# Ipsedo/MARLClassification

Hardware: AMD Instinct MI355X
Metric: agent-env-steps/sec (higher is better)
Workload: dtype f32; 1 GPU; RESISC45 256x256x3, 16 agents, 16 steps, f=12, README dims (configs[2]); full train iteration: rollout + A2C loss + BPTT backward + Adam; batch_per_gpu=256, global_batch=256, parallelism=dp1, rng=library (Philox4x32-10), launch=eager

## Files before the change

marlclassification_amd/csrc/common.h:

```cpp
#pragma once

#include <hip/hip_runtime.h>
#include <stdint.h>
#include <stdio.h>

#include "../../include/marl_hip.h"
#include "../../include/marl_hip_gemmops.h"
#include "split.h"

namespace marl {

constexpr int kWave = 64;

inline int p4(int x) { return (x + 3) & ~3; }
inline int64_t cdiv(int64_t a, int64_t b) { return (a + b - 1) / b; }

void set_error(const char* fmt, ...);

int tune_get(const char* key, int dflt);
int tune_set(const char* key, int value);

__device__ __forceinline__ float rcp_fast(float x) { return __builtin_amdgcn_rcpf(x); }
__device__ __forceinline__ float sigmoid_acc(float x) { return rcp_fast(1.0f + __expf(-x)); }
__device__ __forceinline__ float tanh_fast(float x) { return 1.0f - 2.0f * rcp_fast(1.0f + __expf(2.0f * x)); }
// ... 375 lines not shown
                         const float* c_prev, const float* c_new, int ldc, int64_t rows, int n,
                         hipStream_t st);
struct LstmBwdBatch;
int launch_lstm_cell_bwd_batch(LstmBwdBatch& b, int count, hipStream_t st);
int launch_lstm_cell_bwd2(const float* dh0, int lddh0, float* dc0, int lddc0, float* gates0,
                          int ldg0, const float* cp0, const float* cn0, int ldc0, int n0,
                          const float* dh1, int lddh1, float* dc1, int lddc1, float* gates1,
                          int ldg1, const float* cp1, const float* cn1, int ldc1, int n1,
                          int64_t rows, hipStream_t st);

struct SampleArgs {
    const float* a_pol;
    int ld_a, nla;
    const float* w1;
    int ldw;
    const float* b1;
    const float* noise;
    uint64_t rng_seed, rng_ctr;
    const uint64_t* rng_off_dev;
    int rng_on;
    const int64_t* forced;
    const int32_t* pos_in;
    int32_t* pos_out;
    int64_t* step_pos;
    int64_t* step_actions;
    float* step_logp;
    float* probs;
    int32_t* actions_i32;
    int R, nA, H, W, f;
    int32_t table[MARL_MAX_ACTIONS][2];
    const float* pe_W;
    const float* pe_b;
    const float* pe_gamma;
    const float* pe_beta;
    float* pe_npos;
    float* pe_z;
    float* pe_stats;
    float* pe_out;
    int pe_ldz, pe_ldo, pe_nd;
    char* pe_img;
    int pe_row0, pe_steps, pe_col0;
    float ex_inv_tau, ex_keep, ex_floor;
    int ex_greedy;
};
int launch_sample(const SampleArgs& a, hipStream_t st, bool explore = false);

int launch_draw_episode(uint64_t seed, uint64_t offset, const uint64_t* offset_dev, int64_t* pos0,
                        int R, int H, int W, int f, float* h0, float* c0, int n_b, float* hc0,
                        float* cc0, int n_a, float* noise, int64_t n_noise, hipStream_t st);

struct PermDesc {
    const float* src;
    float* dst;
    int rows, cols;
    int dst_ld;
    int rd, rs1, rs2;
    int cd, cs1, cs2;
    int frag;
    const float* src2;
};
constexpr int kMaxPerm = 56;
struct PermBatch {
    PermDesc d[kMaxPerm];
    int count;
};
int launch_permute(const PermBatch& b, hipStream_t st);

__host__ __device__ inline int panel_frag_groups(int K) { return (K + 15) >> 4; }
__host__ __device__ inline size_t panel_frag_floats(int n, int K) {
    return ((size_t)((n + 31) >> 5) * panel_frag_groups(K) + 3) * 512;
}
__host__ __device__ inline size_t panel_frag_index(int r, int k, int groups) {
    return ((((size_t)(r >> 5) * groups + (k >> 4)) * 2 + ((r >> 4) & 1)) * 64 + ((k >> 2) & 3) * 16 + (r & 15)) * 4 +
           (k & 3);
}

struct Counters {
    uint64_t rng_offset;
    uint64_t step;
    float lr_over_bc1;
    float inv_sqrt_bc2;
    float pad[2];
};
static_assert(sizeof(Counters) == MARL_COUNTERS_BYTES, "counter block layout");
int launch_counters_set(Counters* c, uint64_t rng_offset, int64_t step, float lr, float beta1,
                        float beta2, int tick, hipStream_t st);

int launch_adam(float* p, const float* g, float* m, float* v, int64_t n, float lr_over_bc1,
                float inv_sqrt_bc2, float beta1, float beta2, float eps, float grad_scale,
                hipStream_t st, const Counters* cnt = nullptr);

int launch_fill(float* p, int64_t n, float v, hipStream_t st);
int launch_add2d(const float* a, int64_t lda, const float* b, int64_t ldb, float* out, int64_t ldo,
                 int64_t rows, int cols, hipStream_t st);
int launch_copy2d(const float* src, int64_t lds, float* dst, int64_t ldd, int64_t rows, int cols,
                  hipStream_t st);
int launch_i64_to_i32(const int64_t* src, int32_t* dst, int64_t n, hipStream_t st);
int launch_policy_dlogits(const float* dlogp, const float* probs, const int32_t* actions,
                          float* out, int ld, int64_t rows, int nA, hipStream_t st);
int launch_policy_dlogits_probs(const float* dlogp, const float* dprobs, const float* probs,
                                const int32_t* actions, float* out, int ld, int64_t rows, int nA,
                                hipStream_t st);
int launch_policy_dlogits_explore(const float* dlogp, const float* dprobs, const float* probs,
                                  const int32_t* actions, float* out, int ld, int64_t rows, int nA,
                                  float inv_tau, float keep, float floor, hipStream_t st);
int launch_acc2d(float* dst, int64_t ldd, const float* src, int64_t lds, int64_t rows, int cols,
                 hipStream_t st);
int launch_rowdot(const float* a, int lda, const float* w, const float* b, float* out,
                  int64_t rows, int n, hipStream_t st);

struct PanelLayer {
    const float* wfrag;
    int wgroups;
    const float* bias;
    const float* gamma;
    const float* beta;
    int n;
    float* z;
    int ldz;
    float* stats;
    float* a;
    int lda;
    char* a3;
    int a3_row0, a3_steps, a3_col0;
};
constexpr int kPanelMaxLayers = 4;
struct PanelFwdProb {
    const float* x;
    int ldx, k0;
    int agg_na, agg_nb;
    float* xbar;
    int m, nlayers;
    PanelLayer layer[kPanelMaxLayers];
    int by_batch, g_na, g_nb, agg_at, ld_xbar;
    const float* mix;
    CommGate gate;
};
struct PanelFwdBatch {
    PanelFwdProb p[2];
    int count;
    int off_panel1, off_red, off_part, off_prm;
    int off_mix;
    int has_sample, panel_blocks;
    int epi_prob;
    int ln_narrow_max;
    SampleArgs sample;
#ifdef MARL_KERNEL_TS
    long long* ts;
#endif
};
int panel_chain_supported(int na, int n_msg, int threads);
int panel_supported(int k0, int n0, int n1);
int panel_sample_supported(int n_actions);
int launch_panel_fwd(PanelFwdBatch& b, hipStream_t st, bool explore = false);

struct LstmBwdArgs {
    const float* dh;
    float* dc;
    float* gates;
    const float* c_prev;
    const float* c_new;
    int lddh, lddc, ldg, ldc, n;
    char* g3;
    int g3_row0, g3_steps;
    int skip_f32;
};
struct LstmBwdBatch {
    LstmBwdArgs a[2];
    int64_t rows;
    int vec4;
};
inline bool lstm_bwd_vec4_ok(const LstmBwdArgs& a) {
    return (a.n & 3) == 0 && (a.lddh & 3) == 0 && (a.lddc & 3) == 0 && (a.ldg & 3) == 0 && (a.ldc & 3) == 0;
}
__device__ __forceinline__ void lstm_cell_bwd_at(const LstmBwdArgs& A, int64_t r, int u, float dhv);
__device__ __forceinline__ void lstm_cell_bwd_elem(const LstmBwdArgs& A, int64_t rows, int64_t idx) {
    const int n = A.n;
    if (idx >= rows * n) return;
    const int64_t r = idx / n;
    const int u = (int)(idx % n);
    lstm_cell_bwd_at(A, r, u, A.dh[r * A.lddh + u]);
}
__device__ __forceinline__ void lstm_cell_bwd_at(const LstmBwdArgs& A, int64_t r, int u, float dhv) {
    const int n = A.n;
    float* g = A.gates + r * A.ldg + u;
    const float gi = g[0], gf = g[n], gg = g[2 * n], go = g[3 * n];
    const float tc = tanh_fast(A.c_new[r * A.ldc + u]);
    const float dcv = dhv * go * (1.0f - tc * tc) + A.dc[r * A.lddc + u];
    g[0] = dcv * gg * gi * (1.0f - gi);
    g[n] = dcv * A.c_prev[r * A.ldc + u] * gf * (1.0f - gf);
    g[2 * n] = dcv * gi * (1.0f - gg * gg);
    g[3 * n] = dhv * tc * go * (1.0f - go);
    A.dc[r * A.lddc + u] = dcv * gf;
}

__device__ __forceinline__ void lstm_cell_bwd_at4(const LstmBwdArgs& A, int64_t r, int u, const float (&dhv)[4]) {
    const int n = A.n;
    float* g = A.gates + r * A.ldg + u;
    const float4 gi4 = *reinterpret_cast<const float4*>(g), gf4 = *reinterpret_cast<const float4*>(g + n),
                 gg4 = *reinterpret_cast<const float4*>(g + 2 * n), go4 = *reinterpret_cast<const float4*>(g + 3 * n);
    const float4 cn4 = *reinterpret_cast<const float4*>(A.c_new + r * A.ldc + u),
                 cp4 = *reinterpret_cast<const float4*>(A.c_prev + r * A.ldc + u),
                 dc4 = *reinterpret_cast<const float4*>(A.dc + r * A.lddc + u);
    const float gi[4] = {gi4.x, gi4.y, gi4.z, gi4.w}, gf[4] = {gf4.x, gf4.y, gf4.z, gf4.w};
    const float gg[4] = {gg4.x, gg4.y, gg4.z, gg4.w}, go[4] = {go4.x, go4.y, go4.z, go4.w};
    const float cn[4] = {cn4.x, cn4.y, cn4.z, cn4.w}, cp[4] = {cp4.x, cp4.y, cp4.z, cp4.w};
    const float dcin[4] = {dc4.x, dc4.y, dc4.z, dc4.w};
    float o[5][4];
#pragma unroll
    for (int q = 0; q < 4; ++q) {
        const float tc = tanh_fast(cn[q]);
        const float dcv = dhv[q] * go[q] * (1.0f - tc * tc) + dcin[q];
        o[0][q] = dcv * gg[q] * gi[q] * (1.0f - gi[q]);
        o[1][q] = dcv * cp[q] * gf[q] * (1.0f - gf[q]);
        o[2][q] = dcv * gi[q] * (1.0f - gg[q] * gg[q]);
        o[3][q] = dhv[q] * tc * go[q] * (1.0f - go[q]);
        o[4][q] = dcv * gf[q];
    }
    if (!(A.g3 && A.skip_f32)) {
#pragma unroll
        for (int k = 0; k < 4; ++k)
            *reinterpret_cast<float4*>(g + k * n) = make_float4(o[k][0], o[k][1], o[k][2], o[k][3]);
    }
    *reinterpret_cast<float4*>(A.dc + r * A.lddc + u) = make_float4(o[4][0], o[4][1], o[4][2], o[4][3]);
    if (A.g3) {
#pragma unroll
        for (int k = 0; k < 4; ++k) {
            const int col = k * n + u;
            img_store4(A.g3 + img_off(A.g3_row0 + r, col >> 4, A.g3_steps), col, o[k][0], o[k][1], o[k][2], o[k][3]);
        }
    }
}
__device__ __forceinline__ void lstm_cell_bwd_elem4(const LstmBwdArgs& A, int64_t rows, int64_t idx) {
    const int n4 = A.n >> 2;
    if (idx >= rows * n4) return;
    const int64_t r = idx / n4;
    const int u = (int)(idx - r * n4) * 4;
    const float4 d = *reinterpret_cast<const float4*>(A.dh + r * A.lddh + u);
    const float dhv[4] = {d.x, d.y, d.z, d.w};
    lstm_cell_bwd_at4(A, r, u, dhv);
}

struct PanelBwdLayer {
    const float* z;
    int ldz;
    const float* stats;
    const float* gamma;
    const float* beta;
    int n;
    float* dz;
    int lddz;
    float* part;
    const float* wtfrag;
    int wgroups;
    int k_in;
};
struct PanelBwdProb {
    const float* da;
    int ldda;
    const float* da2;
    int ldda2;
    int agg_na, agg_nb;
    int m, nlayers;
    PanelBwdLayer layer[kPanelMaxLayers];
    float* dx;
    int lddx, accumulate;
    int by_batch, g_na, g_nb, agg_at;
    int has_cellb;
    LstmBwdArgs cellb;
    int off_e, off_prm, off_colp, off_part, off_rowmap;
    const float* mix;
    int off_mix;
    int tail_lds;
    int has_cell, panel_blocks;
    LstmBwdArgs cell;
    int64_t cell_rows;
    int cell_vec4;
    int cellb_img_done, cell_img_done;
    CommGate gate;
#ifdef MARL_KERNEL_TS
    long long* ts;
#endif
};
int panel_bwd_blocks(int m);
int panel_chain_blocks(int na, int nb);
int panel_chain_by_batch(int na);
int launch_panel_bwd(PanelBwdProb& p, hipStream_t st);

#ifdef MARL_KERNEL_TS
constexpr int kTsWaves = 16, kTsSlots = 48, kTsRoles = 2;
#define MARL_TS_DECL(ptr) long long* ts_ = (ptr); int tsi_ = 0
#define MARL_TS()                                                                              \
    if (ts_ && (threadIdx.x & 63) == 0 && blockIdx.x == 37 && blockIdx.y < kTsRoles && tsi_ < kTsSlots) \
    ts_[((int)blockIdx.y * kTsWaves + (threadIdx.x >> 6)) * kTsSlots + tsi_++] = wall_clock64()
int ts_begin(long long** dev, int call);
void ts_report(const char* tag, long long* dev, int waves, int role = 0);
#else
#define MARL_TS_DECL(ptr)
#define MARL_TS()
#endif

struct FDiv {
    uint32_t d, m;
};
inline FDiv make_fdiv(int d) { return FDiv{(uint32_t)d, (uint32_t)(((1ull << 32) / (uint64_t)d) + 1)}; }
__device__ __forceinline__ int fdiv(int n, FDiv f) {
// ... 178 lines not shown
```

marlclassification_amd/csrc/episode.hip:

```cpp
#include <math.h>
#include <stdlib.h>
#include <string.h>

#include "../../include/marl_hip_rowops.h"
#include "../../include/marl_hip_cnnops.h"
#include "../../include/marl_hip_explore.h"
#include "../../include/marl_hip_classloss.h"
#include "../../include/marl_hip_softtargets.h"
#include "common.h"

namespace marl {

struct Dims {
    int na, nb, ns;
    int64_t R, NR;
    int H, W, c_img, f;
    int L;
    int ch[MARL_MAX_CNN_LAYERS + 1];
    int grp[MARL_MAX_CNN_LAYERS];
    int hw[MARL_MAX_CNN_LAYERS + 1];
    int P[MARL_MAX_CNN_LAYERS];
    int K[MARL_MAX_CNN_LAYERS];
    int ldk[MARL_MAX_CNN_LAYERS];
    int nf, nin;
// ... 399 lines not shown
    e.u3_stride_rows = 0;
    e.tn_cell[0] = e.tn_cell[1] = GemmPlan{};
    if (e.g3) {
        e.tn_cell[0] = g3_tn_cell_plan(4 * d.n_b, d.nin, d.n_b, d.NR);
        e.tn_cell[1] = g3_tn_cell_plan(4 * d.n_a, d.nin, d.n_a, d.NR);
        e.u3_stride_rows = train ? R : 0;
        e.U3 = b.take(img_bytes((int64_t)(train ? NR : R), d.nin) / sizeof(float));
        e.H3 = b.take(img_bytes((int64_t)(S1 * R), d.n_b) / sizeof(float));
        e.HC3 = b.take(img_bytes((int64_t)(S1 * R), d.n_a) / sizeof(float));
    }
    if (train && e.g3) {
        e.GB3 = b.take(img_bytes((int64_t)NR, 4 * d.n_b) / sizeof(float));
        e.GA3 = b.take(img_bytes((int64_t)NR, 4 * d.n_a) / sizeof(float));
    }
    if (train) {
        e.GPRED = b.take(NR * d.ld_nC);
        e.DLOG = b.take(NR * d.ld_nA);
        e.DVAL = b.take(NR * 4);
        e.DAQ1 = b.take(NR * d.ld_nlb);
        e.DAC1 = b.take(NR * d.ld_nla);
        e.DAP1 = b.take(NR * d.ld_nla);
        e.DH = b.take(S1 * R * d.ld_nb);
        e.DHC = b.take(S1 * R * d.ld_na);
        e.DC = b.take(R * d.ld_nb);
        e.DCC = b.take(R * d.ld_na);
        e.DDBAR = b.take(NR * d.ld_dbl);
        e.DDBAR2 = b.take(NR * d.ld_dbl);
        e.DAD1 = b.take(NR * d.ld_nm2);
        e.DMBAR = b.take(R * d.ld_nm);
        e.DZE2 = b.take(NR * d.ld_nm);
        e.DAE1 = b.take(NR * d.ld_nm2);
        e.DU = b.take(NR * d.ld_nin);
        e.DZPOS = b.take(NR * d.ld_nd);
        int maxg = 4 * (d.n_b > d.n_a ? d.n_b : d.n_a);
        e.BTMP = b.take((size_t)maxg);
        {
            int blocks = panel_bwd_blocks((int)d.R);
            if (panel_chain_blocks(d.na, d.nb) > blocks) blocks = panel_chain_blocks(d.na, d.nb);
            const size_t nblk = (size_t)blocks * d.ns * 2;
            e.PLN[0] = b.take(nblk * d.n_mo);
            e.PLN[1] = b.take(nblk * d.nm2);
            e.PLN[2] = b.take(nblk * d.n_m);
            e.PLN[3] = b.take(nblk * d.nm2);
        }
        for (int l = 0; l < d.L; ++l) {
            e.DZ[l] = b.take(NR * d.P[l] * d.ch[l + 1]);
            e.DCOLS[l] = (l > 0 && !e.dgrad[l].rb) ? b.take(NR * d.P[l] * d.ldk[l]) : 0;
            e.DA[l] = (l + 1 < d.L && !e.dgrad[l + 1].rb) ? b.take(NR * d.P[l] * d.ch[l + 1]) : 0;
        }
        size_t part = 0, tns = 0, red = 0;
        auto upd_part = [&](int64_t blocks, int n) {
            const size_t v = (size_t)blocks * 2 * n;
            part = v > part ? v : part;
            red += ((v + 63) & ~(size_t)63) + 64 * 2 * (size_t)n + 64;
        };
        auto upd_tn = [&](int ni, int nj, int64_t rows) {
            const size_t v = gemm_tn_scratch_bytes(ni, nj, rows);
            tns = v > tns ? v : tns;
            red += v / sizeof(float) + 64 * ((size_t)ni * nj + ni) + 192;
        };
        const int64_t nr = d.NR, r = d.R;
        upd_part(ln_bwd_blocks(nr, d.nlb), d.nlb);
        upd_part(ln_bwd_blocks(nr, d.nla), d.nla);
        upd_part(ln_bwd_blocks(nr, d.n_d), d.n_d);
        upd_part(ln_bwd_blocks(r, d.nm2), d.nm2);
        upd_part(ln_bwd_blocks(r, d.n_mo), d.n_mo);
        upd_part(ln_bwd_blocks(r, d.n_m), d.n_m);
        for (int l = 0; l < d.L; ++l) upd_part(gn_bwd_blocks(nr, d.ch[l + 1]), d.ch[l + 1]);
        for (int l = 1; l < d.L; ++l)
            if (e.dgrad[l].rb) upd_part(e.dgrad[l].chunks, d.ch[l]);
        upd_tn(d.nC, d.nlb, nr);
        upd_tn(d.nlb, d.n_b, nr);
        upd_tn(1, d.nla, nr);
        upd_tn(d.nla, d.n_a, nr);
        upd_tn(d.nA, d.nla, nr);
        upd_tn(d.n_mo, d.nm2, nr);
        upd_tn(d.nm2, d.n_m, nr);
        upd_tn(d.n_m, d.nm2, nr);
        upd_tn(d.nm2, d.n_b, nr);
        upd_tn(4 * d.n_b, d.nin, nr);
        upd_tn(4 * d.n_b, d.n_b, nr);
        upd_tn(4 * d.n_a, d.nin, nr);
        upd_tn(4 * d.n_a, d.n_a, nr);
        if (e.g3) {
            const int tn3[4][2] = {{4 * d.n_b, d.nin}, {4 * d.n_b, d.n_b}, {4 * d.n_a, d.nin}, {4 * d.n_a, d.n_a}};
            for (const auto& q : tn3) {
                const size_t v = g3_tn_plan(q[0], q[1], nr, false).scratch_bytes;
                tns = v > tns ? v : tns;
            }
            for (const GemmPlan& q : e.tn_cell) tns = q.scratch_bytes > tns ? q.scratch_bytes : tns;
        }
        upd_tn(d.n_d, 2, nr);
        for (int l = 0; l < d.L; ++l) {
            if (e.wgrad[l].form) {
                const size_t v = (size_t)e.wgrad[l].blocks_bound *
                                 ((size_t)d.ch[l + 1] * d.K[l] + d.ch[l + 1]) * sizeof(float);
                tns = v > tns ? v : tns;
                red += v / sizeof(float) + 64 * ((size_t)d.ch[l + 1] * (d.K[l] + 1)) + 192;
            } else {
                upd_tn(d.ch[l + 1], d.K[l], nr * d.P[l]);
            }
        }
        e.part_floats = part;
        e.tns_bytes = tns;
        e.PART = b.take(part);
        e.TNS = b.take(tns / sizeof(float) + 16);
        {
            const int pn[4] = {d.n_mo, d.nm2, d.n_m, d.nm2};
            for (int n : pn) red += 64 * 2 * (size_t)n + 64;
        }
        e.red_floats = red + 4096;
        e.RED = b.take(e.red_floats);
    }
    e.loss_floats = loss_scratch_floats(d.ns, d.na, d.nb);
    e.LOSS = b.take(e.loss_floats);
    e.total = b.off;
}

struct Explore {
    bool on;
    float inv_tau, keep, eps;
    int greedy;
};
struct ClassLoss {
    bool on;
    const float* w;
    int nc;
    float eps;
    const float* sw;
    int ns;
    bool wrew;
};
struct SoftTargets {
    const float* q;
    int nb, nc;
};
struct Installed {
    const float* comm = nullptr;
    int comm_na = 0;
    CommGate range = {nullptr, -1, 0, 1};
    Explore explore = {false, 1.f, 1.f, 0.f, 0};
    ClassLoss class_loss = {false, nullptr, 0, 0.f, nullptr, 0, false};
    SoftTargets soft = {nullptr, 0, 0};
    hipEvent_t heads_event = nullptr;
};
static Installed g_installed;

enum SampleSite { SAMPLE_OWN = 0, SAMPLE_EPILOGUE, SAMPLE_RIDE };
struct Plan {
    bool panels;
    bool panels_bwd;
    bool chain;
    bool panel_sample;
    bool g3_lstm;
    bool g3_tn, g3_tn_pipe;
    bool g3_tn_cell;
    bool u3_by_producers;
    int skip_f32;
    int lstm_plan;
    SampleSite sample;
    int comm_form;
    int explore_form;
    int comm, comm_range, explore, class_loss;
    int soft_targets;
};

struct Ctx {
    Dims d;
    WLayout w;
    ELayout e;
    float* W;
    float* E;
    hipStream_t st;
    int train;
    RedQueue* rq = nullptr;
    TnQueue* tq = nullptr;
    bool defer_slabs = false;
    size_t defer_small = 0;
    bool defer_this(size_t slab_bytes) const { return defer_slabs || (defer_small && slab_bytes <= defer_small); }
    Installed opt;
    Plan plan;
    int u3_row(int t) const { return (int)(e.u3_stride_rows * (size_t)t); }

    const char* wp3k(int i) const { return reinterpret_cast<const char*>(W + w.wp3k[i]); }
    const char* wt3k(int i) const { return reinterpret_cast<const char*>(W + w.wt3k[i]); }
    char* img(size_t off) const { return reinterpret_cast<char*>(E + off); }
    const float* wp(int i) const { return W + w.wp[i]; }
    const float* wt(int i) const { return W + w.wt[i]; }
    GemmB wpB(int i) const {
        const ParamMeta m = param_meta(d, i);
        return GemmB{wp(i), w.ldp[i], m.k, m.kind == PK_MATRIX ? W + w.wp3[i] : nullptr, (m.k + 31) / 32};
    }
    GemmB wtB(int i) const {
        const ParamMeta m = param_meta(d, i);
        return GemmB{wt(i), w.ldt[i], m.n, m.kind == PK_MATRIX ? W + w.wt3[i] : nullptr, (m.n + 31) / 32};
    }
    const float* wpf(int i) const { return w.wpf[i] ? W + w.wpf[i] : nullptr; }
    const float* wtf(int i) const { return w.wtf[i] ? W + w.wtf[i] : nullptr; }
    float* gp(int i) const { return W + w.gp[i]; }
    float* at(size_t off) const { return E + off; }
    float* at(const SBuf& s, int t) const { return E + s.at(train ? t : 0); }
    float* Hs(int t) const { return E + e.H + (size_t)t * d.R * d.ld_nb; }
    float* Cs(int t) const { return E + e.C + (size_t)t * d.R * d.ld_nb; }
    float* HCs(int t) const { return E + e.HC + (size_t)t * d.R * d.ld_na; }
    float* CCs(int t) const { return E + e.CC + (size_t)t * d.R * d.ld_na; }
    float* MSGs(int t) const { return E + e.MSG + (size_t)t * d.R * d.ld_nm; }
    int32_t* POSs(int t) const { return reinterpret_cast<int32_t*>(E + e.POS) + (size_t)t * d.R * 2; }
    float* PROBSs(int t) const { return E + e.PROBS + (size_t)t * d.R * d.nA; }
    int32_t* ACTs(int t) const { return reinterpret_cast<int32_t*>(E + e.ACT) + (size_t)t * d.R; }
    float* DHs(int t) const { return E + e.DH + (size_t)t * d.R * d.ld_nb; }
    float* DHCs(int t) const { return E + e.DHC + (size_t)t * d.R * d.ld_na; }
};

static Plan make_plan(const Dims& d, const WLayout& w, const ELayout& e, const Installed& opt) {
    auto env_on = [](const char* v) { return !(v && v[0] == '0'); };
    static const bool env_panels = env_on(getenv("MARL_PANELS")), env_sample = env_on(getenv("MARL_PANEL_SAMPLE"));
    Plan p{};
    p.panels = env_panels && panel_model_ok(d);
    p.panels_bwd = p.panels && d.n_mo <= 384 && d.nm2 <= 384 && d.n_m <= 384;
    p.chain = p.panels_bwd && panel_chain_supported(d.na, d.n_m, 256) && tune_get("panel_chain", 1) != 0 &&
              (!opt.comm || d.n_b <= 384);
    p.panel_sample = p.chain && env_sample && panel_sample_supported(d.nA);
    p.sample = p.chain ? (p.panel_sample ? SAMPLE_EPILOGUE : SAMPLE_OWN)
                       : (p.panels && !opt.explore.on ? SAMPLE_RIDE : SAMPLE_OWN);
    p.comm_form = opt.comm ? (p.chain ? 5 : p.panels ? 3 : 4) : p.chain ? 0 : p.panels ? 1 : 2;
    p.explore_form = !opt.explore.on ? 0 : p.panel_sample ? 1 : 2;
    p.comm = opt.comm != nullptr;
    p.comm_range = opt.range.radius >= 0 ? opt.range.radius : -1;
    p.explore = opt.explore.on;
    p.class_loss = opt.class_loss.on;
    p.soft_targets = opt.soft.q != nullptr;

    const int k_lstm = tune_get("g3_lstm", 1), k_tn = tune_get("g3_tn", 1);
    p.g3_lstm = e.g3 && k_lstm != 0;
    if (p.g3_lstm) {
        G3Batch b{};
        b.count = 2;
        b.p[0].m = b.p[1].m = (int)d.R;
        b.p[0].n = d.n_b;
        b.p[1].n = d.n_a;
        p.lstm_plan = g3_lstm_plan(b).variant;
    }
    p.g3_tn = p.g3_lstm && k_tn != 0 &&
              (k_tn == 2 || (d.nin <= 640 && d.n_b <= 512 && d.n_a <= 512 &&
                             (d.NR >= 32768 || (e.tn_cell[0].ok && e.tn_cell[1].ok))));
    p.g3_tn_cell = p.g3_tn && e.tn_cell[0].ok && e.tn_cell[1].ok;
    p.g3_tn_pipe = p.g3_tn && e.tn_cell[0].pipelined;
    p.skip_f32 = p.panels_bwd && p.g3_tn;
    p.u3_by_producers = p.g3_lstm && e.fwd.writes_image && p.panels &&
                        ((d.nf | d.n_mo | d.n_d) & 3) == 0 &&
                        d.nin % 16 == 0;
    return p;
}

static int make_ctx(const marl_config* cfg, const void* wws, size_t wbytes, void* ews, size_t ebytes,
                    int train, void* stream, Ctx& c) {
    MARL_TRY(make_dims(cfg, c.d));
    c.opt = g_installed;
    if (c.opt.comm && c.opt.comm_na != c.d.na) {
        set_error("communication matrix is %d x %d but the configuration has %d agents", c.opt.comm_na,
                  c.opt.comm_na, c.d.na);
        return MARL_EINVAL;
    }
    if (c.opt.range.radius >= 0 && !c.opt.comm) {
        set_error("a communication range is installed without its base matrix (marl_comm_matrix)");
        return MARL_EINVAL;
    }
    make_wlayout(c.d, c.w);
    make_elayout(c.d, c.w, train, c.e);
    if (wbytes < c.w.total * sizeof(float) || ebytes < c.e.total * sizeof(float)) {
        set_error("workspace too small for the current configuration / tuning knobs: weights %zu of %zu "
                  "bytes, episode %zu of %zu bytes (ask marl_workspace_sizes again)", wbytes,
                  c.w.total * sizeof(float), ebytes, c.e.total * sizeof(float));
        return MARL_ESIZE;
    }
    c.W = const_cast<float*>(static_cast<const float*>(wws));
    c.E = static_cast<float*>(ews);
    c.st = static_cast<hipStream_t>(stream);
    c.train = train;
    if (!c.W || !c.E) {
        set_error("null workspace");
        return MARL_EINVAL;
    }
    if ((reinterpret_cast<uintptr_t>(c.W) & 255) || (reinterpret_cast<uintptr_t>(c.E) & 255)) {
        set_error("workspaces must be 256-byte aligned");
        return MARL_EINVAL;
    }
    c.plan = make_plan(c.d, c.w, c.e, c.opt);
    return MARL_OK;
}

static int gemm1(const Ctx& c, const GemmProb& p) {
    GemmBatch b{};
    b.p[0] = p;
    b.count = 1;
    return launch_gemm_nt(b, c.st);
}
static int gemm2(const Ctx& c, const GemmProb& p0, const GemmProb& p1) {
    GemmBatch b{};
    b.p[0] = p0;
    b.p[1] = p1;
    b.count = 2;
    return launch_gemm_nt(b, c.st);
}

struct StepIn {
    const float* obs = nullptr;
    const float* npos = nullptr;
    const void* img = nullptr;
    int img_u8 = 0;
};

struct CnnFwdIo {
    const void* img = nullptr;
    const float* obs = nullptr;
    const int32_t* pos = nullptr;
    int img_u8 = 0;
    int64_t rows = 0;
    float* cols[MARL_MAX_CNN_LAYERS] = {};
    float* z[MARL_MAX_CNN_LAYERS] = {};
    float* gst[MARL_MAX_CNN_LAYERS] = {};
    float* u = nullptr;
    int ldu = 0;
    char* u3 = nullptr;
    int u3_row0 = 0, u3_steps = 0;
};
static CnnFwdArgs cnn_fwd_args(const Dims& d, const WLayout& w, const float* W, const CnnFwdIo& io) {
    CnnFwdArgs a{};
    a.img = io.img;
    a.obs = io.obs;
    a.pos = io.pos;
    a.img_u8 = io.img_u8;
    a.rows = io.rows;
    a.nb = d.nb;
    a.c_img = d.c_img;
    a.H = d.H;
    a.W = d.W;
    a.f = d.f;
    a.L = d.L;
    for (int l = 0; l < d.L; ++l)
        a.layer[l] = CnnFwdLayer{W + w.wp[4 * l], W + w.wp[4 * l + 1], W + w.wp[4 * l + 2], W + w.wp[4 * l + 3],
                                 io.cols[l], io.z[l], io.gst[l],
                                 d.ch[l], d.ch[l + 1], d.grp[l], d.hw[l], d.hw[l + 1], d.P[l],
                                 d.K[l], d.ldk[l], w.wf[4 * l] ? W + w.wf[4 * l] : nullptr};
    a.u = io.u;
    a.ldu = io.ldu;
    a.u3 = io.u3;
    a.u3_row0 = io.u3_row0;
    a.u3_steps = io.u3_steps;
    return a;
}


static int step_cnn(const Ctx& c, int t, const StepIn& in) {
    const Dims& d = c.d;
    hipStream_t st = c.st;
    if (c.e.fwd.which) {
        CnnFwdIo io;
        io.img = in.img;
        io.obs = in.obs;
        io.pos = c.POSs(t);
        io.img_u8 = in.img_u8;
        io.rows = d.R;
        for (int l = 0; l < d.L; ++l) {
            io.cols[l] = c.e.keeps_cols[l] ? c.at(c.e.COLS[l], t) : nullptr;
            io.z[l] = c.train ? c.at(c.e.Z[l], t) : nullptr;
            io.gst[l] = c.train ? c.at(c.e.GST[l], t) : nullptr;
        }
        io.u = c.at(c.e.U, t);
        io.ldu = d.ld_nin;
        if (c.plan.u3_by_producers) {
            io.u3 = c.img(c.e.U3);
            io.u3_row0 = c.u3_row(t);
            io.u3_steps = img_steps(d.nin);
        }
// ... 1865 lines not shown
                       size_t step_ws_bytes, const float* obs, const float* g_probs, const float* g_logp,
                       const float* g_values, const float* g_preds, const float* g_msg, const float* g_h,
                       const float* g_c, const float* g_hc, const float* g_cc, float* const* grads_host,
                       float* d_msg, float* d_h, float* d_c, float* d_hc, float* d_cc, void* stream) {
    if (!cfg) {
        set_error("step_backward: null configuration");
        return MARL_EINVAL;
    }
    if (g_installed.range.radius >= 0) {
        set_error("step_backward: a communication range is installed - a single step has no integer positions of "
                  "the emission step; run the fused episode");
        return MARL_EINVAL;
    }
    marl_config one = *cfg;
    one.nb_steps = 1;
    Ctx c;
    MARL_TRY(make_ctx(&one, weights_ws, weights_ws_bytes, step_ws, step_ws_bytes, 1, stream, c));
    if (!grads_host || !obs) {
        set_error("step_backward: null gradient table or observation");
        return MARL_EINVAL;
    }
    StepBwd sb;
    sb.obs = obs;
    sb.g_probs = g_probs;
    sb.g_msg = g_msg;
    sb.g_h = g_h;
    sb.g_c = g_c;
    sb.g_hc = g_hc;
    sb.g_cc = g_cc;
    sb.d_msg = d_msg;
    sb.d_h = d_h;
    sb.d_c = d_c;
    sb.d_hc = d_hc;
    sb.d_cc = d_cc;
    return episode_backward(c, nullptr, 0, g_preds, g_logp, g_values, grads_host, &sb);
}

int marl_debug_buffer(const marl_config* cfg, int train, const char* name, int t,
                      int64_t* offset_floats, int* ld) {
    Dims d;
    MARL_TRY(make_dims(cfg, d));
    WLayout w;
    make_wlayout(d, w);
    ELayout e;
    make_elayout(d, w, train, e);
    if (!name || !offset_floats || !ld || t < 0 || t > d.ns) return MARL_EINVAL;
    const size_t R = (size_t)d.R;
    const int ts = train ? t : 0;
    auto set = [&](size_t off, int l) {
        *offset_floats = (int64_t)off;
        *ld = l;
        return MARL_OK;
    };
    if (!strncmp(name, "WP", 2) || !strncmp(name, "WT", 2)) {
        const int idx = atoi(name + 2);
        if (name[2] == 'F') {
            const int fi = atoi(name + 3);
            const size_t off = fi >= 0 && fi < MARL_NPARAMS ? (name[1] == 'P' ? w.wpf[fi] : w.wtf[fi]) : 0;
            if (!off) {
                set_error("parameter %d has no fragment-order copy", fi);
                return MARL_EINVAL;
            }
            return set(off, name[1] == 'P' ? w.gpf[fi] : w.gtf[fi]);
        }
        if (idx < 0 || idx >= MARL_NPARAMS || param_meta(d, idx).kind == PK_NONE) {
            set_error("no parameter %d", idx);
            return MARL_EINVAL;
        }
        return name[1] == 'P' ? set(w.wp[idx], w.ldp[idx]) : set(w.wt[idx], w.ldt[idx]);
    }
    if (!strcmp(name, "U")) return set(e.U.at(ts), d.ld_nin);
    if (!strcmp(name, "H")) return set(e.H + (size_t)t * R * d.ld_nb, d.ld_nb);
    if (!strcmp(name, "C")) return set(e.C + (size_t)t * R * d.ld_nb, d.ld_nb);
    if (!strcmp(name, "HC")) return set(e.HC + (size_t)t * R * d.ld_na, d.ld_na);
    if (!strcmp(name, "CC")) return set(e.CC + (size_t)t * R * d.ld_na, d.ld_na);
    if (!strcmp(name, "MSG")) return set(e.MSG + (size_t)t * R * d.ld_nm, d.ld_nm);
    if (!strcmp(name, "PROBS")) return set(e.PROBS + (size_t)t * R * d.nA, d.nA);
    if (!strcmp(name, "COLS0")) {
        if (e.fwd.which && !e.keeps_cols[0]) {
            set_error("COLS0 is not materialised for this shape (fused CNN kernels)");
            return MARL_EINVAL;
        }
        return set(e.COLS[0].at(e.COLS[0].stride ? ts : 0), d.ldk[0]);
    }
    if (!strcmp(name, "Z0")) return set(e.Z[0].at(ts), d.ch[1]);
    if (!strcmp(name, "GB")) return set(e.GB.at(ts), d.ld_gb);
    if (train) {
        if (!strcmp(name, "DU")) return set(e.DU + (size_t)t * R * d.ld_nin, d.ld_nin);
        if (!strcmp(name, "DH")) return set(e.DH + (size_t)t * R * d.ld_nb, d.ld_nb);
        if (!strcmp(name, "DHC")) return set(e.DHC + (size_t)t * R * d.ld_na, d.ld_na);
    }
    set_error("unknown debug buffer %s", name);
    return MARL_EINVAL;
}

int marl_plan_query(const marl_config* cfg, int train, const char* key, int* value) {
    Dims d;
    MARL_TRY(make_dims(cfg, d));
    if (!key || !value) return MARL_EINVAL;
    WLayout w;
    make_wlayout(d, w);
    ELayout e;
    make_elayout(d, w, train, e);
    const Plan plan = make_plan(d, w, e, g_installed);
    if (!strcmp(key, "g3")) *value = e.g3;
    else if (!strcmp(key, "g3_model")) *value = g3_model_ok(d);
    else if (!strcmp(key, "g3_lstm")) *value = plan.g3_lstm;
    else if (!strcmp(key, "g3_tn")) *value = plan.g3_tn;
    else if (!strcmp(key, "lstm_plan")) *value = plan.lstm_plan;
    else if (!strcmp(key, "small_r")) *value = plan.lstm_plan == 3 || plan.lstm_plan == 4;
    else if (!strcmp(key, "g3_tn_cell"))
        *value = plan.g3_tn_cell;
    else if (!strcmp(key, "g3_tn_pipe")) *value = plan.g3_tn_pipe;
    else if (!strcmp(key, "wgrad3")) {
        *value = 0;
        for (int l = 0; l < d.L; ++l)
            if (e.wgrad[l].form == 3) *value = 1;
    }
    else if (!strncmp(key, "cnn_fwd", 7)) {
        const CnnFwdPlan& p = e.fwd;
        if (!strcmp(key, "cnn_fwd")) *value = p.which;
        else if (!strcmp(key, "cnn_fwd_rb")) *value = p.rb;
        else if (!strcmp(key, "cnn_fwd_blocks")) *value = p.blocks;
        else {
            set_error("unknown plan key %s", key);
            return MARL_EINVAL;
        }
    }
    else if (!strncmp(key, "cnn_dgrad_rb", 12) || !strncmp(key, "cnn_wgrad_", 10)) {
        const bool dg = key[4] == 'd';
        const char* rest = key + (dg ? 12 : 10);
        int field = 0;
        if (!dg) {
            if (!strncmp(rest, "rb", 2)) field = 1, rest += 2;
            else if (!strncmp(rest, "chunks", 6)) field = 2, rest += 6;
            else if (!strncmp(rest, "blocks", 6)) field = 3, rest += 6;
        }
        const int l = (rest[0] >= '0' && rest[0] <= '9' && !rest[1]) ? rest[0] - '0' : -1;
        if ((!dg && !field) || l < (dg ? 1 : 0) || l >= d.L) {
            set_error("unknown plan key %s (layers %d..%d)", key, dg ? 1 : 0, d.L - 1);
            return MARL_EINVAL;
        }
        if (dg)
            *value = e.dgrad[l].rb;
        else {
            const CnnWgradPlan& p = e.wgrad[l];
            *value = field == 1 ? p.rb : field == 2 ? p.chunks : p.blocks;
        }
    }
    else if (!strcmp(key, "comm")) *value = plan.comm;
    else if (!strcmp(key, "comm_range")) *value = plan.comm_range;
    else if (!strcmp(key, "panel_chain")) *value = plan.chain;
    else if (!strcmp(key, "panel_sample")) *value = plan.panel_sample;
    else if (!strcmp(key, "explore")) *value = plan.explore;
    else if (!strcmp(key, "class_loss")) *value = plan.class_loss;
    else if (!strcmp(key, "soft_targets")) *value = plan.soft_targets;
    else if (!strcmp(key, "explore_form")) *value = plan.explore_form;
    else if (!strcmp(key, "comm_form")) *value = plan.comm_form;
    else {
        set_error("unknown plan key %s", key);
        return MARL_EINVAL;
    }
    return MARL_OK;
}

}
namespace marl {
__global__ void normalize_positions_kernel(const int64_t* __restrict__ pos, float* __restrict__ out,
                                           int rows, int H, int W) {
    const int r = blockIdx.x * blockDim.x + threadIdx.x;
    if (r >= rows) return;
    out[r * 2] = (float)pos[r * 2] / (float)H;
    out[r * 2 + 1] = (float)pos[r * 2 + 1] / (float)W;
}
}
extern "C" {

int marl_normalize_positions(const int64_t* pos, float* out, int rows, int h, int w, void* stream) {
    if (!pos || !out || rows < 1 || h < 1 || w < 1) {
        set_error("normalize_positions: bad argument");
        return MARL_EINVAL;
    }
    hipLaunchKernelGGL(normalize_positions_kernel, dim3((unsigned)cdiv(rows, 256)), dim3(256), 0,
                       static_cast<hipStream_t>(stream), pos, out, rows, h, w);
    MARL_LAUNCH_CHECK();
    return MARL_OK;
}

int marl_profile_begin(int kernel_class, int max_launches) {
    if (kernel_class < 0 || kernel_class >= kProfClasses || max_launches < 1) return MARL_EINVAL;
    return profile_begin(kernel_class, max_launches);
}
int marl_profile_end(double* total_ms, int* launches) { return profile_end(total_ms, launches); }

int marl_gemm_nt(const float* a, int lda, const float* b, int ldb, const float* bias, float* c,
                 int ldc, int m, int n, int k, int accumulate, void* stream) {
    GemmBatch bt{};
    bt.p[0] = gemm_prob(a, lda, gemm_b(b, ldb, k), c, ldc, m, n, bias, accumulate);
    bt.count = 1;
    return launch_gemm_nt(bt, static_cast<hipStream_t>(stream));
}

size_t marl_gemm_weight_image_bytes(int n, int k) { return split_image_floats(n, k) * sizeof(float); }

int marl_gemm_nt_weights(const float* a, int lda, const float* b, int ldb, const float* bias, float* c,
                         int ldc, int m, int n, int k, int accumulate, void* image_scratch, void* stream) {
    if (!b || !image_scratch || n < 1 || k < 1 || ldb < k) {
        set_error("gemm_nt_weights: bad argument");
        return MARL_EINVAL;
    }
    hipStream_t st = static_cast<hipStream_t>(stream);
    SplitBatch sb{};
    sb.d[0] = SplitDesc{b, image_scratch, n, k, ldb, (k + 31) / 32};
    sb.count = 1;
    MARL_TRY(launch_split_weights(sb, st));
    GemmBatch bt{};
    bt.p[0] = gemm_prob(a, lda, GemmB{b, ldb, k, image_scratch, (k + 31) / 32}, c, ldc, m, n, bias, accumulate);
    bt.count = 1;
    return launch_gemm_nt(bt, st);
}

size_t marl_gemm_tn_scratch(int ni, int nj, int64_t rows) { return gemm_tn_scratch_bytes(ni, nj, rows); }

int marl_gemm_tn(const float* a, int lda, const float* b, int ldb, float* c, int ldc, int ni, int nj,
                 int64_t rows, float* scratch, size_t scratch_bytes, void* stream) {
    return launch_gemm_tn(a, lda, b, ldb, c, ldc, ni, nj, rows, scratch, scratch_bytes,
                          static_cast<hipStream_t>(stream));
}

static CnnWgradArgs wgrad_api_args(int64_t rows, int nb, int c_img, int h, int w, int cin, int cout,
                                   int hin, int groups, int first) {
    CnnWgradArgs g{};
    g.rows = rows;
    g.first = first;
    g.nb = nb;
    g.c_img = c_img;
    g.H = h;
    g.W = w;
    g.cin = cin;
    g.cout = cout;
    g.hin = hin;
    g.hout = (hin - 1) / 2 + 1;
    g.P = g.hout * g.hout;
    g.G = groups > 0 ? groups : 1;
    g.K = 9 * cin;
    return g;
}

size_t marl_cnn_wgrad_scratch(int64_t rows, int cin, int cout, int hin, int groups, int first) {
    CnnWgradArgs g = wgrad_api_args(rows, 1, cin, hin + 1, hin + 1, cin, cout, hin, groups, first);
    return (size_t)cnn_wgrad_plan(g).blocks_bound * ((size_t)cout * 9 * cin + cout) * sizeof(float);
}

int marl_cnn_wgrad(const float* dz, const void* img, int img_u8, const int32_t* pos,
                   const float* zin, const float* gst, const float* gamma, const float* beta,
                   int64_t rows, int nb, int c_img, int h, int w, int cin, int cout, int hin,
                   int groups, float* dw, float* db, float* scratch, size_t scratch_bytes,
                   void* stream) {
    const int first = zin == nullptr;
    if (!dz || !dw || !db || !scratch || rows < 1 || cin < 1 || cout < 1 || hin < 1 ||
        (first ? (!img || !pos || nb < 1) : (!gst || !gamma || !beta))) {
        set_error("cnn_wgrad: bad argument");
        return MARL_EINVAL;
    }
    CnnWgradArgs g = wgrad_api_args(rows, nb, c_img, h, w, cin, cout, hin, groups, first);
    const CnnWgradPlan plan = cnn_wgrad_plan(g);
    if (!plan.form) {
        set_error("cnn_wgrad: shape outside the kernel's range (cin %d cout %d hin %d)", cin, cout, hin);
        return MARL_ELIMIT;
    }
    if (scratch_bytes < (size_t)plan.blocks_bound * ((size_t)cout * 9 * cin + cout) * sizeof(float)) {
        set_error("cnn_wgrad: scratch too small");
        return MARL_ESIZE;
    }
    g.dz = dz;
    g.img = img;
    g.img_u8 = img_u8;
    g.pos = pos;
    g.zin = zin;
    g.gst = gst;
    g.gamma = gamma;
    g.beta = beta;
    g.part_w = scratch;
    hipStream_t st = static_cast<hipStream_t>(stream);
    MARL_TRY(launch_cnn_wgrad(g, st));
    return launch_slab_reduce(g.part_w, (int64_t)cout * g.K, g.blocks, dw, g.K, cout, g.K, g.part_b, db, st);
}

int marl_tune(const char* key, int value) {
    if (!key) return MARL_EINVAL;
    return tune_set(key, value);
}

int marl_tune_get(const char* key, int dflt) { return key ? tune_get(key, dflt) : dflt; }

int marl_ln_silu_fwd(const float* z, int ldz, const float* gamma, const float* beta, float* out,
                     int ldo, float* stats, int m, int n, void* stream) {
    return launch_ln_silu_fwd(z, ldz, gamma, beta, out, ldo, stats, m, n,
                              static_cast<hipStream_t>(stream));
}

int marl_ln_silu_bwd(const float* da, int ldda, const float* g, int ldg, int kin, const float* w1t, int ldw,
                     const float* z, int ldz, const float* stats, const float* gamma, const float* beta,
                     float* dz, int lddz, float* dgamma, float* dbeta, float* scratch, size_t scratch_bytes,
                     int m, int n, void* stream) {
    if (!z || !stats || !gamma || !beta || !dz || !dgamma || !dbeta || !scratch || m < 0 || n < 1 ||
// ... 209 lines not shown
```

marlclassification_amd/csrc/panel.hip:

```cpp
#include <stdlib.h>

#include "common.h"
#include "sample.h"

namespace marl {

typedef float f32x4 __attribute__((ext_vector_type(4)));

__device__ __forceinline__ void lds_barrier() {
    asm volatile("s_waitcnt lgkmcnt(0)\n\ts_barrier" ::: "memory");
}
__device__ __forceinline__ float silu_p(float y) { return silu_fast(y); }
__device__ __forceinline__ float silu_grad_p(float y) { return silu_grad_fast(y); }

constexpr int kPanelRows = 16;
constexpr int kPanelMaxWaves = 12;
constexpr int kPanelMaxCols = 6;

__host__ __device__ inline int panel_stride(int k) { return ((k + 15) & ~15) + 4; }

__device__ __forceinline__ void panel_gemm(f32x4 (&acc)[2], const float* in, int stride,
                                           const float* __restrict__ wfrag, int groups, int j,
                                           int kbeg, int kend, int lane) {
    const int quad = lane >> 4, l16 = lane & 15;
    const float* arow = in + l16 * stride + 4 * quad;
    const int g0 = __builtin_amdgcn_readfirstlane(j * groups + (kbeg >> 4));
    const float* wb = wfrag + (size_t)g0 * 512;
    const unsigned lo = 4u * (unsigned)lane;
#pragma unroll
    for (int r = 0; r < 4; ++r) acc[0][r] = acc[1][r] = 0.f;
    for (int k0 = kbeg; k0 < kend; k0 += 64, wb += 4 * 512) {
        float4 b0[4], b1[4];
#pragma unroll
        for (int i = 0; i < 4; ++i) {
            b0[i] = *reinterpret_cast<const float4*>(wb + 512 * i + lo);
            b1[i] = *reinterpret_cast<const float4*>(wb + 512 * i + 256 + lo);
        }
#pragma unroll
        for (int i = 0; i < 4; ++i) {
            if (k0 + 16 * i < kend) {
                const float4 a = *reinterpret_cast<const float4*>(arow + k0 + 16 * i);
                acc[0] = __builtin_amdgcn_mfma_f32_16x16x4f32(a.x, b0[i].x, acc[0], 0, 0, 0);
                acc[1] = __builtin_amdgcn_mfma_f32_16x16x4f32(a.x, b1[i].x, acc[1], 0, 0, 0);
                acc[0] = __builtin_amdgcn_mfma_f32_16x16x4f32(a.y, b0[i].y, acc[0], 0, 0, 0);
                acc[1] = __builtin_amdgcn_mfma_f32_16x16x4f32(a.y, b1[i].y, acc[1], 0, 0, 0);
                acc[0] = __builtin_amdgcn_mfma_f32_16x16x4f32(a.z, b0[i].z, acc[0], 0, 0, 0);
                acc[1] = __builtin_amdgcn_mfma_f32_16x16x4f32(a.z, b1[i].z, acc[1], 0, 0, 0);
                acc[0] = __builtin_amdgcn_mfma_f32_16x16x4f32(a.w, b0[i].w, acc[0], 0, 0, 0);
                acc[1] = __builtin_amdgcn_mfma_f32_16x16x4f32(a.w, b1[i].w, acc[1], 0, 0, 0);
            }
        }
    }
}

__device__ __forceinline__ void panel_ksum(f32x4 (&acc)[2], float* part, int nt, int ks, int j, int s,
                                           int lane, bool active) {
    if (ks > 1) {
        if (active && s > 0) {
            float* p = part + ((size_t)((s - 1) * nt + j) * 64 + lane) * 8;
            *reinterpret_cast<float4*>(p) = make_float4(acc[0][0], acc[0][1], acc[0][2], acc[0][3]);
            *reinterpret_cast<float4*>(p + 4) = make_float4(acc[1][0], acc[1][1], acc[1][2], acc[1][3]);
        }
        lds_barrier();
        if (active && s == 0) {
            for (int q = 1; q < ks; ++q) {
                const float* p = part + ((size_t)((q - 1) * nt + j) * 64 + lane) * 8;
                const float4 u = *reinterpret_cast<const float4*>(p);
                const float4 v = *reinterpret_cast<const float4*>(p + 4);
                acc[0][0] += u.x;
                acc[0][1] += u.y;
                acc[0][2] += u.z;
                acc[0][3] += u.w;
                acc[1][0] += v.x;
                acc[1][1] += v.y;
                acc[1][2] += v.z;
                acc[1][3] += v.w;
            }
        }
    }
}

__host__ __device__ inline int panel_ksplit(int K, int nt, int nwaves) {
    const int K16 = (K + 15) & ~15;
    int ks = nwaves / nt;
    const int want = (K16 + 63) / 64;
    ks = ks < want ? ks : want;
    return ks < 1 ? 1 : ks;
}

template <int NC>
__device__ __forceinline__ void panel_ln_rows(const PanelLayer& Lr, float* outp, int ys, int n, const float* lgamma,
                                              const float* lbeta, const int* rowmap, int wave, int nwaves, int lane)
{
    constexpr int RPW = 4;
    float g[NC], bt[NC];
#pragma unroll
    for (int u = 0; u < NC; ++u) {
        const int c = lane + 64 * u;
        g[u] = c < n ? lgamma[c] : 0.f;
        bt[u] = c < n ? lbeta[c] : 0.f;
    }
    const float inv_n = 1.0f / (float)n;
#pragma unroll
    for (int i = 0; i < RPW; ++i) {
        const int lr = wave + i * nwaves;
        if (lr < kPanelRows) {
            float* zr = outp + lr * ys;
            const int row = rowmap[lr];
            float v[NC];
            float sm = 0.f;
#pragma unroll
            for (int u = 0; u < NC; ++u) {
                const int c = lane + 64 * u;
                v[u] = c < n ? zr[c] : 0.f;
                sm += v[u];
                if (Lr.z && row >= 0 && c < n) Lr.z[(size_t)row * Lr.ldz + c] = v[u];
            }
            const float mean = wave_sum(sm) * inv_n;
            float q = 0.f;
#pragma unroll
            for (int u = 0; u < NC; ++u) {
                const int c = lane + 64 * u;
                const float d = c < n ? v[u] - mean : 0.f;
                v[u] = d;
                q += d * d;
            }
            const float rstd = 1.0f / sqrtf(wave_sum(q) * inv_n + 1e-5f);
            float* arow = Lr.a + (size_t)(row < 0 ? 0 : row) * Lr.lda;
#pragma unroll
            for (int u = 0; u < NC; ++u) {
                const int c = lane + 64 * u;
                if (c < n) {
                    const float av = silu_p(v[u] * rstd * g[u] + bt[u]);
                    zr[c] = av;
                    if (row >= 0) arow[c] = av;
                }
            }
            if (Lr.stats && lane == 0 && row >= 0) {
                Lr.stats[(size_t)row * 2] = mean;
                Lr.stats[(size_t)row * 2 + 1] = rstd;
            }
            if (Lr.a3 && row >= 0) {
                for (int c4 = 4 * lane; c4 < n; c4 += 256) {
                    const float4 t = *reinterpret_cast<const float4*>(zr + c4);
                    const int col = Lr.a3_col0 + c4;
                    img_store4(Lr.a3 + img_off((int64_t)Lr.a3_row0 + row, col >> 4, Lr.a3_steps), col, t.x, t.y, t.z, t.w);
                }
            }
        }
    }
}

template <int MAXA, bool UNI, bool EXPLORE = false>
__device__ __forceinline__ void panel_sample_rows(const SampleArgs& A0, const float* outp, int ys, const int* rowmap,
                                                  int wave, int nwaves, int lane) {
    for (int lr = __builtin_amdgcn_readfirstlane(wave); lr < kPanelRows; lr += nwaves) {
        const int row = __builtin_amdgcn_readfirstlane(rowmap[lr]);
        if (row < 0) continue;
        int ln = (int)__builtin_amdgcn_mbcnt_hi(~0u, __builtin_amdgcn_mbcnt_lo(~0u, 0u));
        asm volatile("" : "+v"(ln));
        int zero = 0;
        asm volatile("" : "+s"(zero));
        const SampleArgs& A = (&A0)[zero];
        float p[MAXA];
        SamplePre<MAXA> S;
        sample_prefetch_row<MAXA>(A, row, ln, S);
        sample_row_logits_at<MAXA, kPanelMaxCols>(A, outp + lr * ys, p, ln);
        if (UNI) {
            auto uni = [](float v) { return __int_as_float(__builtin_amdgcn_readfirstlane(__float_as_int(v))); };
#pragma unroll
            for (int j = 0; j < MAXA; ++j) {
                S.b1[j] = uni(S.b1[j]);
                S.nz[j] = uni(S.nz[j]);
            }
            S.ctr = ((uint64_t)(uint32_t)__builtin_amdgcn_readfirstlane((int)(S.ctr >> 32)) << 32) |
                    (uint32_t)__builtin_amdgcn_readfirstlane((int)S.ctr);
            S.pi0 = __builtin_amdgcn_readfirstlane(S.pi0);
            S.pi1 = __builtin_amdgcn_readfirstlane(S.pi1);
            S.forced = __builtin_amdgcn_readfirstlane(S.forced);
        }
        sample_prefetch_pe<MAXA>(A, ln, S);
        sample_finish<MAXA, EXPLORE>(A, row, p, ln, S);
    }
}

template <int SAMPLE, bool MIX = false, bool EPI = false, bool GATE = false, bool EXPLORE = false>
__global__ __launch_bounds__(768, 6) void panel_fwd_kernel(const PanelFwdBatch B) {
    extern __shared__ __attribute__((aligned(16))) float lds[];
    if (!EPI && SAMPLE > 0 && (int)blockIdx.x >= B.panel_blocks) {
        const int r = ((int)blockIdx.x - B.panel_blocks) * (int)(blockDim.x >> 6) + (int)(threadIdx.x >> 6);
        if (r >= B.sample.R) return;
        constexpr int MAXA = SAMPLE > 0 ? SAMPLE : 4;
        float p[MAXA];
        SamplePre<MAXA> S;
        sample_prefetch<MAXA, false>(B.sample, r, threadIdx.x & 63, S);
        sample_row_logits<MAXA>(B.sample, r, p, threadIdx.x & 63);
        sample_finish<MAXA>(B.sample, r, p, threadIdx.x & 63, S);
        return;
    }
    const PanelFwdProb& P = B.p[blockIdx.y];
    const int m0 = blockIdx.x * kPanelRows;
    const int bpb = P.by_batch;
    if (bpb ? (int)blockIdx.x * bpb >= P.g_nb : m0 >= P.m) return;
    const int tid = threadIdx.x, lane = tid & 63, wave = tid >> 6, nwaves = blockDim.x >> 6;
    int* rowmap = reinterpret_cast<int*>(lds + B.off_red);
    if (tid < kPanelRows) {
        int r = m0 + tid < P.m ? m0 + tid : -1;
        if (bpb) {
            const int a = tid / bpb, b = (int)blockIdx.x * bpb + (tid - a * bpb);
            r = (a < P.g_na && b < P.g_nb) ? a * P.g_nb + b : -1;
        }
        rowmap[tid] = r;
    }
    lds_barrier();
    const int quad = lane >> 4, l16 = lane & 15;
#ifdef MARL_KERNEL_TS
    MARL_TS_DECL(B.ts);
#endif
    MARL_TS();
    float* X = lds;
    float* Y = lds + B.off_panel1;
    float* part = lds + B.off_part;
    float* prm = lds + B.off_prm;
    float pv[kPanelMaxLayers][3];
#pragma unroll
    for (int l = 0; l < kPanelMaxLayers; ++l) {
        pv[l][0] = pv[l][1] = pv[l][2] = 0.f;
        if (l < P.nlayers && tid < P.layer[l].n) {
            pv[l][0] = P.layer[l].bias[tid];
            pv[l][1] = P.layer[l].gamma[tid];
            pv[l][2] = P.layer[l].beta[tid];
        }
    }
    float cmv = 0.f;
    if (MIX && !GATE && P.mix && tid < P.g_na * P.g_na) cmv = P.mix[tid];
    if (MIX && GATE && tid < bpb * P.g_na * P.g_na) {
        const int na = P.g_na, i = tid / (na * na), e = tid - i * na * na, a = e / na;
        const int b = (int)blockIdx.x * bpb + i;
        if (b < P.g_nb) cmv = comm_gate_weight<kPanelRows>(P.mix, P.gate, na, P.g_nb, b, a, e - a * na);
    }

    {
        const int k0 = P.k0, xs = panel_stride(k0), K16 = (k0 + 15) & ~15;
        const int c4 = K16 >> 2;
        const int K4 = (k0 + 3) & ~3;
        if (!GATE && P.agg_na > 0) {
            const int na = P.agg_na, nb = P.agg_nb;
            const float den = (float)(na - 1);
            for (int e = tid; e < kPanelRows * c4; e += blockDim.x) {
                const int lr = e / c4, k = (e % c4) * 4;
                const int r = rowmap[lr];
                float4 v = make_float4(0.f, 0.f, 0.f, 0.f);
                if (r >= 0 && k < K4 && na > 1) {
                    const int b = r % nb;
                    const float* base = P.x + (size_t)b * P.ldx + k;
                    const size_t astr = (size_t)nb * P.ldx;
                    float4 s = make_float4(0.f, 0.f, 0.f, 0.f);
                    for (int a0 = 0; a0 < na; a0 += 8) {
                        float4 qv[8];
#pragma unroll
                        for (int u = 0; u < 8; ++u) {
                            const int a = a0 + u < na ? a0 + u : na - 1;
                            qv[u] = *reinterpret_cast<const float4*>(base + (size_t)a * astr);
                        }
#pragma unroll
                        for (int u = 0; u < 8; ++u) {
                            if (a0 + u < na) {
                                s.x += qv[u].x;
                                s.y += qv[u].y;
                                s.z += qv[u].z;
                                s.w += qv[u].w;
                            }
                        }
                    }
                    const float4 me = *reinterpret_cast<const float4*>(P.x + (size_t)r * P.ldx + k);
                    v = make_float4((s.x - me.x) / den, (s.y - me.y) / den, (s.z - me.z) / den,
                                    (s.w - me.w) / den);
                    if (P.xbar) *reinterpret_cast<float4*>(P.xbar + (size_t)r * P.ldx + k) = v;
                }
                *reinterpret_cast<float4*>(X + lr * xs + k) = v;
            }
        } else {
            float4 xv[2];
#pragma unroll
            for (int it = 0; it < 2; ++it) {
                const int e = tid + it * (int)blockDim.x;
                xv[it] = make_float4(0.f, 0.f, 0.f, 0.f);
                if (e < kPanelRows * c4) {
                    const int lr = e / c4, k = (e % c4) * 4;
                    const int r = rowmap[lr];
                    if (r >= 0 && k < K4) xv[it] = *reinterpret_cast<const float4*>(P.x + (size_t)r * P.ldx + k);
                }
            }
#pragma unroll
            for (int it = 0; it < 2; ++it) {
                const int e = tid + it * (int)blockDim.x;
                if (e < kPanelRows * c4) {
                    const int lr = e / c4, k = (e % c4) * 4;
                    *reinterpret_cast<float4*>(X + lr * xs + k) = xv[it];
                }
            }
            for (int e = tid + 2 * (int)blockDim.x; e < kPanelRows * c4; e += blockDim.x) {
                const int lr = e / c4, k = (e % c4) * 4;
                const int r = rowmap[lr];
                float4 v = make_float4(0.f, 0.f, 0.f, 0.f);
                if (r >= 0 && k < K4) v = *reinterpret_cast<const float4*>(P.x + (size_t)r * P.ldx + k);
                *reinterpret_cast<float4*>(X + lr * xs + k) = v;
            }
        }
    }
    {
        int off = 0;
#pragma unroll
        for (int l = 0; l < kPanelMaxLayers; ++l) {
            if (l < P.nlayers) {
                const int n = P.layer[l].n;
                if (tid < n) {
                    prm[off + tid] = pv[l][0];
                    prm[off + n + tid] = pv[l][1];
                    prm[off + 2 * n + tid] = pv[l][2];
                }
                off += 3 * n;
            }
        }
    }
    if (MIX && !GATE && P.mix && tid < P.g_na * P.g_na) lds[B.off_mix + tid] = cmv;
    if (MIX && GATE && tid < bpb * P.g_na * P.g_na) lds[B.off_mix + tid] = cmv;
    MARL_TS();
    lds_barrier();
    MARL_TS();

    int prm_off = 0, K = P.k0;
    for (int l = 0; l < P.nlayers; ++l) {
        const PanelLayer Lr = P.layer[l];
        const float* lbias = prm + prm_off;
        const float* lgamma = lbias + Lr.n;
        const float* lbeta = lgamma + Lr.n;
        prm_off += 3 * Lr.n;
        float* in = (l & 1) ? Y : X;
        float* outp = (l & 1) ? X : Y;
        const int K16 = (K + 15) & ~15;
        const int stride = panel_stride(K);
        if (l > 0 && l == P.agg_at) {
            const int c4 = K16 >> 2, K4 = (K + 3) & ~3, na = P.g_na;
            const float den = (float)(na - 1);
            float4 v[2];
#pragma unroll
            for (int it = 0; it < 2; ++it) {
                const int e = tid + it * (int)blockDim.x;
                v[it] = make_float4(0.f, 0.f, 0.f, 0.f);
                if (e < kPanelRows * c4) {
                    const int lr = e / c4, k = (e - lr * c4) * 4;
                    const int a = lr / bpb, i = lr - a * bpb;
                    if (MIX) {
                        if (a < na) {
                            const float* crow = lds + B.off_mix + (GATE ? i * na + a : a) * na;
                            float4 sm = make_float4(0.f, 0.f, 0.f, 0.f);
                            for (int a2 = 0; a2 < na; ++a2) {
                                const float cf = crow[a2];
                                if (cf != 0.f) {
                                    const float4 q = *reinterpret_cast<const float4*>(in + (a2 * bpb + i) * stride + k);
                                    sm.x = fmaf(cf, q.x, sm.x);
                                    sm.y = fmaf(cf, q.y, sm.y);
                                    sm.z = fmaf(cf, q.z, sm.z);
                                    sm.w = fmaf(cf, q.w, sm.w);
                                }
                            }
                            v[it] = sm;
                        }
                    } else if (a < na && na > 1) {
                        float4 sm = make_float4(0.f, 0.f, 0.f, 0.f);
                        for (int a2 = 0; a2 < na; ++a2) {
                            const float4 q = *reinterpret_cast<const float4*>(in + (a2 * bpb + i) * stride + k);
                            sm.x += q.x;
                            sm.y += q.y;
                            sm.z += q.z;
                            sm.w += q.w;
                        }
                        const float4 me = *reinterpret_cast<const float4*>(in + lr * stride + k);
                        v[it] = make_float4((sm.x - me.x) / den, (sm.y - me.y) / den, (sm.z - me.z) / den,
                                            (sm.w - me.w) / den);
                    }
                }
            }
            lds_barrier();
#pragma unroll
            for (int it = 0; it < 2; ++it) {
                const int e = tid + it * (int)blockDim.x;
                if (e < kPanelRows * c4) {
                    const int lr = e / c4, k = (e - lr * c4) * 4;
                    *reinterpret_cast<float4*>(in + lr * stride + k) = v[it];
                    const int r = rowmap[lr];
                    if (r >= 0 && k < K4 && P.xbar)
                        *reinterpret_cast<float4*>(P.xbar + (size_t)r * P.ld_xbar + k) = v[it];
                }
            }
            lds_barrier();
        }
        const int n = Lr.n, nt = (n + 31) >> 5;
        const int ks = panel_ksplit(K, nt, nwaves);
        const int j = wave % nt, s = wave / nt;
        const bool active = s < ks;
        const int kper = (((K16 + ks - 1) / ks) + 15) & ~15;
        const int kbeg = s * kper;
        const int kend = kbeg + kper < K16 ? kbeg + kper : K16;
        f32x4 acc[2];
        if (active) panel_gemm(acc, in, stride, Lr.wfrag, Lr.wgroups, j, kbeg, kend, lane);
        MARL_TS();
        panel_ksum(acc, part, nt, ks, j, s, lane, active);
        MARL_TS();

        const int ys = panel_stride(n), n16 = (n + 15) & ~15;
        if (active && s == 0) {
#pragma unroll
            for (int t = 0; t < 2; ++t) {
                const int col = j * 32 + 16 * t + l16;
                const bool cv = col < n;
                const float bv = cv ? lbias[col] : 0.f;
#pragma unroll
                for (int r = 0; r < 4; ++r) {
                    const int lr = 4 * quad + r;
                    const float zv = cv ? acc[t][r] + bv : 0.f;
                    if (col < n16) outp[lr * ys + col] = zv;
                }
            }
        }
        MARL_TS();
        lds_barrier();
        MARL_TS();
        if (n <= B.ln_narrow_max)
            panel_ln_rows<2>(Lr, outp, ys, n, lgamma, lbeta, rowmap, wave, nwaves, lane);
        else
            panel_ln_rows<kPanelMaxCols>(Lr, outp, ys, n, lgamma, lbeta, rowmap, wave, nwaves, lane);
        MARL_TS();
        lds_barrier();
        MARL_TS();
        K = n;
    }
    if (EPI && (int)(&P - B.p) + 1 == B.epi_prob) {
        constexpr int MAXA = SAMPLE > 0 ? SAMPLE : 4;
        panel_sample_rows<MAXA, MIX || EXPLORE, EXPLORE>(B.sample, (P.nlayers & 1) ? Y : X, panel_stride(K), rowmap, wave, nwaves, lane);
        MARL_TS();
    }
}

constexpr size_t kPanelMaxLds = 144 * 1024;

static int panel_waves_for(int k, int n) {
    const int nt = (n + 31) / 32;
    const int want = (((k + 15) & ~15) + 63) / 64;
    int w = nt * want;
    if (w < nt) w = nt;
    return w > kPanelMaxWaves ? (nt > kPanelMaxWaves ? -1 : (kPanelMaxWaves / nt) * nt) : w;
}

int panel_chain_supported(int na, int n_msg, int threads) {
    const int K16 = (n_msg + 15) & ~15;
    return na >= 1 && na <= kPanelRows && kPanelRows * (K16 / 4) <= 2 * threads;
}

int panel_sample_supported(int n_actions) { return n_actions >= 1 && n_actions <= 4; }

int panel_supported(int k0, int n0, int n1) {
    if (n0 > 32 * kPanelMaxWaves || n1 > 32 * kPanelMaxWaves) return 0;
    if (n0 > 64 * kPanelMaxCols || n1 > 64 * kPanelMaxCols) return 0;
    const int kx = k0 > n1 ? k0 : n1;
    const size_t lds = (size_t)(kPanelRows * panel_stride(kx) + kPanelRows * panel_stride(n0) +
                                (kPanelMaxWaves + 1) * 32 + (kPanelMaxWaves - 1) * 512 +
                                3 * (n0 + n1) + 16) * 4;
    return lds <= kPanelMaxLds;
}

static int panel_kper_host(int K16, int ks) { return (((K16 + ks - 1) / ks) + 15) & ~15; }

struct PanelFwdPlan {
    int waves;
    size_t lds;
    unsigned pblocks;
    bool mixed, gated;
};
static int panel_fwd_plan(PanelFwdBatch& b, PanelFwdPlan& pl) {
    int waves = 1, x0 = 0, x1 = 0;
    for (int i = 0; i < b.count; ++i) {
        const PanelFwdProb& p = b.p[i];
        for (int l = 0; l < p.nlayers; ++l) {
            const int kin = l == 0 ? p.k0 : p.layer[l - 1].n;
            if (!p.layer[l].wfrag) {
                set_error("panel kernel: layer %d has no fragment-order weight copy", l);
                return MARL_EINVAL;
            }
            if (p.layer[l].wgroups != panel_frag_groups(kin)) {
                set_error("panel kernel: layer %d's weight copy has %d K groups, its input width %d needs %d", l,
                          p.layer[l].wgroups, kin, panel_frag_groups(kin));
                return MARL_ELIMIT;
            }
            const int w = panel_waves_for(kin, p.layer[l].n);
            if (w < 0) {
                set_error("panel kernel: layer width %d too large", p.layer[l].n);
                return MARL_ELIMIT;
            }
            waves = w > waves ? w : waves;
        }
        int s0 = kPanelRows * panel_stride(p.k0), s1 = 0;
        for (int l = 0; l < p.nlayers; ++l) {
            const int v = kPanelRows * panel_stride(p.layer[l].n);
            if (l & 1)
                s0 = v > s0 ? v : s0;
            else
                s1 = v > s1 ? v : s1;
        }
        if (p.agg_at > 0 && (p.by_batch < 1 || p.g_na * p.by_batch > kPanelRows || p.agg_at >= p.nlayers ||
                             !panel_chain_supported(p.g_na, p.layer[p.agg_at - 1].n, 256))) {
            set_error("panel kernel: in-panel message mean outside its range");
            return MARL_ELIMIT;
        }
        if (p.mix && (p.agg_at <= 0 || i != 0 || (b.has_sample && b.count == 1))) {
            set_error("panel kernel: a mixing matrix needs the in-panel aggregation of problem 0");
            return MARL_ELIMIT;
        }
        if ((p.gate.pos && (!p.mix || p.by_batch * p.g_na * p.g_na > kPanelRows * kPanelRows)) ||
            (b.p[0].gate.pos && p.agg_na > 0)) {
            set_error("panel kernel: a position gate needs a base matrix, no staged mean and by_batch * agents^2 <= %d",
                      kPanelRows * kPanelRows);
            return MARL_ELIMIT;
        }
        x0 = s0 > x0 ? s0 : x0;
        x1 = s1 > x1 ? s1 : x1;
    }
    const bool mixed = b.count > 0 && b.p[0].mix != nullptr;
    const bool gated = mixed && b.p[0].gate.pos != nullptr;
    if (waves < 4) waves = 4;
    b.off_panel1 = x0;
    b.off_red = x0 + x1;
    b.off_part = b.off_red + (kPanelMaxWaves + 1) * 32;
    b.off_prm = b.off_part + (waves - 1) * 512;
    int prm = 0;
    for (int i = 0; i < b.count; ++i) {
        int q = 0;
        for (int l = 0; l < b.p[i].nlayers; ++l) q += 3 * b.p[i].layer[l].n;
        prm = q > prm ? q : prm;
    }
    b.off_mix = b.off_prm + prm + 16;
    const size_t lds = (size_t)(b.off_mix + (mixed ? kPanelRows * kPanelRows : 0)) * sizeof(float);
    if (lds > kPanelMaxLds) {
        set_error("panel kernel: shape outside its range");
        return MARL_ELIMIT;
    }
    b.ln_narrow_max = 128;
    unsigned pblocks = 0;
    for (int i = 0; i < b.count; ++i) {
        const PanelFwdProb& p = b.p[i];
        const unsigned nblk = p.by_batch > 0 ? (unsigned)cdiv(p.g_nb, p.by_batch) : (unsigned)cdiv(p.m, kPanelRows);
        pblocks = nblk > pblocks ? nblk : pblocks;
    }
    pl.waves = waves;
    pl.lds = lds;
    pl.pblocks = pblocks;
    pl.mixed = mixed;
    pl.gated = gated;
    return MARL_OK;
}

int launch_panel_fwd(PanelFwdBatch& b, hipStream_t st, bool explore) {
    PanelFwdPlan pl;
    MARL_TRY(panel_fwd_plan(b, pl));
    const int waves = pl.waves;
    const size_t lds = pl.lds;
    const unsigned pblocks = pl.pblocks;
    const bool mixed = pl.mixed, gated = pl.gated;
    static bool raised = false;
    if (!raised) {
        const void* kerns[11] = {reinterpret_cast<const void*>(panel_fwd_kernel<0>),
                                reinterpret_cast<const void*>(panel_fwd_kernel<4>),
                                reinterpret_cast<const void*>(panel_fwd_kernel<MARL_MAX_ACTIONS>),
                                reinterpret_cast<const void*>(panel_fwd_kernel<0, true>),
                                reinterpret_cast<const void*>(panel_fwd_kernel<4, false, true>),
                                reinterpret_cast<const void*>(panel_fwd_kernel<4, true, true>),
                                reinterpret_cast<const void*>(panel_fwd_kernel<0, true, false, true>),
                                reinterpret_cast<const void*>(panel_fwd_kernel<4, true, true, true>),
                                reinterpret_cast<const void*>(panel_fwd_kernel<4, false, true, false, true>),
                                reinterpret_cast<const void*>(panel_fwd_kernel<4, true, true, false, true>),
                                reinterpret_cast<const void*>(panel_fwd_kernel<4, true, true, true, true>)};
        for (const void* kf : kerns)
            MARL_HIP_CHECK(hipFuncSetAttribute(kf, hipFuncAttributeMaxDynamicSharedMemorySize, (int)kPanelMaxLds));
        raised = true;
    }
#ifdef MARL_KERNEL_TS
    static long long* d_ts = nullptr;
    static int calls = 0;
    const int rec = ts_begin(&d_ts, calls++);
    b.ts = rec ? d_ts : nullptr;
#endif
    if (b.epi_prob) {
        const PanelFwdProb* p = b.epi_prob >= 1 && b.epi_prob <= b.count ? &b.p[b.epi_prob - 1] : nullptr;
        if (!p || !panel_sample_supported(b.sample.nA) || p->nlayers < 1 || p->m != b.sample.R ||
            p->layer[p->nlayers - 1].a != b.sample.a_pol || p->layer[p->nlayers - 1].n != b.sample.nla) {
            set_error("panel kernel: the sampling epilogue needs the problem whose last layer writes its activations");
            return MARL_EINVAL;
        }
    }
    if (explore && !b.epi_prob) {
        set_error("panel kernel: exploration controls are served by the sampling epilogue only");
        return MARL_EINVAL;
    }
    for (int i = 0; i < b.count; ++i) {
        const PanelFwdProb& p = b.p[i];
        if (p.agg_na == 1 && p.xbar) {
            PermBatch z{};
            z.count = 1;
            z.d[0].dst = p.xbar, z.d[0].rows = p.m, z.d[0].cols = (p.k0 + 3) & ~3, z.d[0].dst_ld = p.ldx;
            z.d[0].rd = z.d[0].cd = 1;
            MARL_TRY(launch_permute(z, st));
        }
    }
    prof_before(4, st);
    if (b.epi_prob && explore) {
        b.has_sample = 0;
        if (gated)
            hipLaunchKernelGGL((panel_fwd_kernel<4, true, true, true, true>), dim3(pblocks, (unsigned)b.count),
                               dim3(64 * waves), lds, st, b);
        else if (mixed)
            hipLaunchKernelGGL((panel_fwd_kernel<4, true, true, false, true>), dim3(pblocks, (unsigned)b.count),
                               dim3(64 * waves), lds, st, b);
        else
            hipLaunchKernelGGL((panel_fwd_kernel<4, false, true, false, true>), dim3(pblocks, (unsigned)b.count),
                               dim3(64 * waves), lds, st, b);
    } else if (b.epi_prob) {
        b.has_sample = 0;
        if (gated)
            hipLaunchKernelGGL((panel_fwd_kernel<4, true, true, true>), dim3(pblocks, (unsigned)b.count),
                               dim3(64 * waves), lds, st, b);
        else if (mixed)
            hipLaunchKernelGGL((panel_fwd_kernel<4, true, true>), dim3(pblocks, (unsigned)b.count), dim3(64 * waves),
                               lds, st, b);
        else
            hipLaunchKernelGGL((panel_fwd_kernel<4, false, true>), dim3(pblocks, (unsigned)b.count), dim3(64 * waves),
                               lds, st, b);
    } else if (b.has_sample && b.count == 1) {
        b.panel_blocks = (int)pblocks;
        const unsigned sblocks = (unsigned)cdiv(b.sample.R, waves);
        if (b.sample.nA <= 4)
            hipLaunchKernelGGL(panel_fwd_kernel<4>, dim3(pblocks + sblocks, 1), dim3(64 * waves), lds, st, b);
        else
            hipLaunchKernelGGL(panel_fwd_kernel<MARL_MAX_ACTIONS>, dim3(pblocks + sblocks, 1), dim3(64 * waves), lds, st, b);
    } else {
        b.has_sample = 0;
        if (gated)
            hipLaunchKernelGGL((panel_fwd_kernel<0, true, false, true>), dim3(pblocks, (unsigned)b.count),
                               dim3(64 * waves), lds, st, b);
        else if (mixed)
            hipLaunchKernelGGL((panel_fwd_kernel<0, true>), dim3(pblocks, (unsigned)b.count), dim3(64 * waves),
                               lds, st, b);
        else
            hipLaunchKernelGGL(panel_fwd_kernel<0>, dim3(pblocks, (unsigned)b.count), dim3(64 * waves), lds, st, b);
    }
    prof_after(4, st);
    MARL_LAUNCH_CHECK();
#ifdef MARL_KERNEL_TS
    if (rec) {
        fprintf(stderr, "[ts] panel_fwd count %d sample %d epilogue %d waves %d lds %zu\n", b.count, b.has_sample,
                b.epi_prob, waves, lds);
        ts_report("panel_fwd", d_ts, waves);
        if (b.count == 2) ts_report("panel_fwd role 1", d_ts, waves, 1);
    }
#endif
    return MARL_OK;
}

constexpr int kBwdMaxCols = kPanelMaxCols;

template <bool CELL, int MAXC, bool MIX = false, bool GATE = false>
__global__ __launch_bounds__(768, 4) void panel_bwd_kernel(const PanelBwdProb P) {
    extern __shared__ __attribute__((aligned(16))) float lds[];
    if (CELL && (int)blockIdx.x >= P.panel_blocks) {
        const int64_t idx = (int64_t)((int)blockIdx.x - P.panel_blocks) * blockDim.x + threadIdx.x;
        if (P.cell_vec4)
            lstm_cell_bwd_elem4(P.cell, P.cell_rows, idx);
        else
            lstm_cell_bwd_elem(P.cell, P.cell_rows, idx);
        return;
    }
    const int m0 = blockIdx.x * kPanelRows;
    const int bpb = P.by_batch;
    if (bpb ? (int)blockIdx.x * bpb >= P.g_nb : m0 >= P.m) return;
    const int tid = threadIdx.x, lane = tid & 63, wave = tid >> 6, nwaves = blockDim.x >> 6;
    const int quad = lane >> 4, l16 = lane & 15;
    float* D = lds;
    float* E = lds + P.off_e;
    float* prm = lds + P.off_prm;
    float* colp = lds + P.off_colp;
    float* part = lds + P.off_part;
    int* rowmap = reinterpret_cast<int*>(lds + P.off_rowmap);
    if (tid < kPanelRows) {
        int r = m0 + tid < P.m ? m0 + tid : -1;
        if (bpb) {
            const int a = tid / bpb, b = (int)blockIdx.x * bpb + (tid - a * bpb);
            r = (a < P.g_na && b < P.g_nb) ? a * P.g_nb + b : -1;
        }
        rowmap[tid] = r;
    }
    lds_barrier();
#ifdef MARL_KERNEL_TS
    MARL_TS_DECL(P.ts);
#endif
    MARL_TS();

    float zpre[2][MAXC], mpre[2], rpre[2];
    auto zfetch = [&](const PanelBwdLayer& L) {
#pragma unroll
        for (int i = 0; i < 2; ++i) {
            const int lr = wave + i * nwaves;
            const int row = lr < kPanelRows ? rowmap[lr] : -1;
            const size_t rr = row < 0 ? 0 : (size_t)row;
            mpre[i] = L.stats[rr * 2];
            rpre[i] = L.stats[rr * 2 + 1];
#pragma unroll
            for (int u = 0; u < MAXC; ++u) {
                const int c = lane + 64 * u;
                zpre[i][u] = c < L.n ? L.z[rr * L.ldz + c] : 0.f;
            }
        }
    };
    zfetch(P.layer[0]);
    {
        float pv[kPanelMaxLayers][2];
#pragma unroll
        for (int l = 0; l < kPanelMaxLayers; ++l) {
            pv[l][0] = pv[l][1] = 0.f;
            if (l < P.nlayers && tid < P.layer[l].n) {
                pv[l][0] = P.layer[l].gamma[tid];
                pv[l][1] = P.layer[l].beta[tid];
            }
        }
        float cmv = 0.f;
        if (MIX && !GATE && tid < P.g_na * P.g_na) {
            const int a = tid / P.g_na, a2 = tid - a * P.g_na;
            cmv = P.mix[a2 * P.g_na + a];
        }
        if (MIX && GATE && tid < bpb * P.g_na * P.g_na) {
            const int na = P.g_na, i = tid / (na * na), e = tid - i * na * na, a = e / na;
            const int b = (int)blockIdx.x * bpb + i;
            if (b < P.g_nb) cmv = comm_gate_weight<kPanelRows>(P.mix, P.gate, na, P.g_nb, b, e - a * na, a);
        }
        int off = 0;
#pragma unroll
        for (int l = 0; l < kPanelMaxLayers; ++l) {
            if (l < P.nlayers) {
                const int n = P.layer[l].n;
                if (tid < n) {
                    prm[off + tid] = pv[l][0];
                    prm[off + n + tid] = pv[l][1];
                }
                off += 2 * n;
            }
        }
        if (MIX && !GATE && tid < P.g_na * P.g_na) lds[P.off_mix + tid] = cmv;
        if (MIX && GATE && tid < bpb * P.g_na * P.g_na) lds[P.off_mix + tid] = cmv;
        const int n = P.layer[0].n, ds = panel_stride(n), n16 = (n + 15) & ~15, c4 = n16 >> 2;
        const int n4 = (n + 3) & ~3;
        for (int e = tid; e < kPanelRows * c4; e += blockDim.x) {
            const int lr = e / c4, k = (e % c4) * 4;
            const int r = rowmap[lr];
            float4 v = make_float4(0.f, 0.f, 0.f, 0.f);
            if (r >= 0 && k < n4 && P.agg_na > 1) {
                const int na = P.agg_na, nb = P.agg_nb;
                const float den = (float)(na - 1);
                const float* base = P.da + (size_t)(r % nb) * P.ldda + k;
                const size_t astr = (size_t)nb * P.ldda;
                float4 s = make_float4(0.f, 0.f, 0.f, 0.f);
                for (int a0 = 0; a0 < na; a0 += 8) {
                    float4 qv[8];
#pragma unroll
                    for (int u = 0; u < 8; ++u) {
                        const int a = a0 + u < na ? a0 + u : na - 1;
                        qv[u] = *reinterpret_cast<const float4*>(base + (size_t)a * astr);
                    }
#pragma unroll
                    for (int u = 0; u < 8; ++u) {
                        if (a0 + u < na) {
                            s.x += qv[u].x;
                            s.y += qv[u].y;
                            s.z += qv[u].z;
                            s.w += qv[u].w;
                        }
                    }
                }
                const float4 me = *reinterpret_cast<const float4*>(P.da + (size_t)r * P.ldda + k);
                v = make_float4((s.x - me.x) / den, (s.y - me.y) / den, (s.z - me.z) / den,
                                (s.w - me.w) / den);
            } else if (r >= 0 && k < n4 && P.agg_na == 0) {
                v = *reinterpret_cast<const float4*>(P.da + (size_t)r * P.ldda + k);
                if (P.da2) {
                    const float4 w = *reinterpret_cast<const float4*>(P.da2 + (size_t)r * P.ldda2 + k);
                    v = make_float4(v.x + w.x, v.y + w.y, v.z + w.z, v.w + w.w);
                }
            }
            *reinterpret_cast<float4*>(D + lr * ds + k) = v;
        }
    }
    MARL_TS();
    lds_barrier();
    MARL_TS();

    int prm_off = 0;
    for (int l = 0; l < P.nlayers; ++l) {
        const PanelBwdLayer Lr = P.layer[l];
        const int n = Lr.n, ds = panel_stride(n), n16 = (n + 15) & ~15;
        const float* lgamma = prm + prm_off;
        const float* lbeta = lgamma + n;
        prm_off += 2 * n;
        if (l > 0 && l == P.agg_at) {
            const int c4 = n16 >> 2, na = P.g_na;
            const float den = (float)(na - 1);
            float4 v[2];
#pragma unroll
            for (int it = 0; it < 2; ++it) {
                const int e = tid + it * (int)blockDim.x;
                v[it] = make_float4(0.f, 0.f, 0.f, 0.f);
                if (e < kPanelRows * c4) {
                    const int lr = e / c4, k = (e - lr * c4) * 4;
                    const int a = lr / bpb, i = lr - a * bpb;
                    if (MIX) {
                        if (a < na) {
                            const float* crow = lds + P.off_mix + (GATE ? i * na + a : a) * na;
                            float4 sm = make_float4(0.f, 0.f, 0.f, 0.f);
                            for (int a2 = 0; a2 < na; ++a2) {
                                const float cf = crow[a2];
                                if (cf != 0.f) {
                                    const float4 q = *reinterpret_cast<const float4*>(D + (a2 * bpb + i) * ds + k);
                                    sm.x = fmaf(cf, q.x, sm.x);
                                    sm.y = fmaf(cf, q.y, sm.y);
                                    sm.z = fmaf(cf, q.z, sm.z);
                                    sm.w = fmaf(cf, q.w, sm.w);
                                }
                            }
                            v[it] = sm;
                        }
                    } else if (a < na && na > 1) {
                        float4 sm = make_float4(0.f, 0.f, 0.f, 0.f);
                        for (int a2 = 0; a2 < na; ++a2) {
                            const float4 q = *reinterpret_cast<const float4*>(D + (a2 * bpb + i) * ds + k);
                            sm.x += q.x;
                            sm.y += q.y;
                            sm.z += q.z;
                            sm.w += q.w;
                        }
                        const float4 me = *reinterpret_cast<const float4*>(D + lr * ds + k);
                        v[it] = make_float4((sm.x - me.x) / den, (sm.y - me.y) / den, (sm.z - me.z) / den,
                                            (sm.w - me.w) / den);
                    }
                }
            }
            lds_barrier();
#pragma unroll
            for (int it = 0; it < 2; ++it) {
                const int e = tid + it * (int)blockDim.x;
                if (e < kPanelRows * c4) {
                    const int lr = e / c4, k = (e - lr * c4) * 4;
                    *reinterpret_cast<float4*>(D + lr * ds + k) = v[it];
                }
            }
            lds_barrier();
        }
        {
            constexpr int RPW = 2;
            float pg[MAXC], pb[MAXC], g[MAXC], bt[MAXC];
#pragma unroll
            for (int u = 0; u < MAXC; ++u) {
                const int c = lane + 64 * u;
                pg[u] = pb[u] = 0.f;
                g[u] = c < n ? lgamma[c] : 0.f;
                bt[u] = c < n ? lbeta[c] : 0.f;
            }
            const float inv_n = 1.0f / (float)n;
#pragma unroll
            for (int i = 0; i < RPW; ++i) {
                const int lr = wave + i * nwaves;
                if (lr < kPanelRows) {
                    const int row = rowmap[lr];
                    const bool rv = row >= 0;
                    float xh[MAXC], dxh[MAXC];
                    float s1 = 0.f, s2 = 0.f, rstd = 0.f;
                    if (rv) {
                        const float mean = mpre[i];
                        rstd = rpre[i];
#pragma unroll
                        for (int u = 0; u < MAXC; ++u) {
                            const int c = lane + 64 * u;
                            xh[u] = dxh[u] = 0.f;
                            if (c < n) {
                                xh[u] = (zpre[i][u] - mean) * rstd;
                                const float dy = D[lr * ds + c] * silu_grad_p(g[u] * xh[u] + bt[u]);
                                dxh[u] = dy * g[u];
                                s1 += dxh[u];
                                s2 += dxh[u] * xh[u];
                                pg[u] += dy * xh[u];
                                pb[u] += dy;
                            }
                        }
                    } else {
#pragma unroll
                        for (int u = 0; u < MAXC; ++u) xh[u] = dxh[u] = 0.f;
                    }
                    const float m1 = wave_sum(s1) * inv_n, m2 = wave_sum(s2) * inv_n;
#pragma unroll
                    for (int u = 0; u < MAXC; ++u) {
                        const int c = lane + 64 * u;
                        if (c < n16) {
                            float dzv = 0.f;
                            if (rv && c < n) {
                                dzv = rstd * (dxh[u] - m1 - xh[u] * m2);
                                Lr.dz[(size_t)row * Lr.lddz + c] = dzv;
                            }
                            D[lr * ds + c] = dzv;
                        }
                    }
                }
            }
            float* cw = colp + (size_t)wave * 2 * n;
#pragma unroll
            for (int u = 0; u < MAXC; ++u) {
                const int c = lane + 64 * u;
                if (c < n) {
                    cw[c] = pg[u];
                    cw[n + c] = pb[u];
                }
            }
        }
        MARL_TS();
        lds_barrier();
        MARL_TS();
        for (int c = tid; c < 2 * n; c += blockDim.x) {
            float t = 0.f;
            for (int w = 0; w < nwaves; ++w) t += colp[(size_t)w * 2 * n + c];
            Lr.part[(size_t)blockIdx.x * 2 * n + c] = t;
        }
        if (l + 1 < P.nlayers) zfetch(P.layer[l + 1]);
        MARL_TS();
        const int nout = Lr.k_in, nt = (nout + 31) >> 5;
        const int ks = panel_ksplit(n, nt, nwaves);
        const int kper = (((n16 + ks - 1) / ks) + 15) & ~15;
        const bool last = l + 1 == P.nlayers;
        const int es = panel_stride(nout), o16 = (nout + 15) & ~15;
        for (int t0 = 0; t0 < nt; t0 += nwaves / ks) {
            const int tiles_round = nwaves / ks;
            const int j = t0 + wave % tiles_round, s = wave / tiles_round;
            const bool active = s < ks && j < nt;
            const int kbeg = s * kper;
            const int kend = kbeg + kper < n16 ? kbeg + kper : n16;
            f32x4 acc[2];
            if (active) panel_gemm(acc, D, ds, Lr.wtfrag, Lr.wgroups, j, kbeg, kend, lane);
            panel_ksum(acc, part, tiles_round, ks, wave % tiles_round, s, lane, active);
            if (active && s == 0) {
                int rw[4];
#pragma unroll
                for (int r = 0; r < 4; ++r) rw[r] = last ? rowmap[4 * quad + r] : -1;
#pragma unroll
                for (int t = 0; t < 2; ++t) {
                    const int col = j * 32 + 16 * t + l16;
#pragma unroll
                    for (int r = 0; r < 4; ++r) {
                        const int lr = 4 * quad + r;
                        const int row = rw[r];
                        const float v = col < nout ? acc[t][r] : 0.f;
                        if (last && P.tail_lds) {
                            if (col < o16) E[lr * es + col] = v;
                        } else if (last) {
                            if (col < nout && row >= 0) {
                                float* o = P.dx + (size_t)row * P.lddx + col;
                                const float tot = P.accumulate ? *o + v : v;
                                *o = tot;
                                if (P.has_cellb) lstm_cell_bwd_at(P.cellb, row, col, tot);
                            }
                        } else if (col < o16) {
                            E[lr * es + col] = v;
                        }
                    }
                }
            }
            lds_barrier();
        }
        MARL_TS();
        if (last && P.tail_lds) {
            const LstmBwdArgs& Cb = P.cellb;
            const int c4n = nout >> 2, items = kPanelRows * c4n, cn = Cb.n;
            constexpr int kIt = 1;
            for (int base = 0; base < items; base += kIt * (int)blockDim.x) {
                float4 ov[kIt], gi[kIt], gf[kIt], gg[kIt], go[kIt], cnew[kIt], cprev[kIt], dcv[kIt];
                int rowi[kIt], coli[kIt], lri[kIt];
#pragma unroll
                for (int k = 0; k < kIt; ++k) {
                    const int i = base + tid + k * (int)blockDim.x;
                    const int lr = i < items ? i / c4n : 0;
                    const int c = i < items ? (i - lr * c4n) * 4 : 0;
                    const int row = i < items ? rowmap[lr] : -1;
                    const size_t rr = row < 0 ? 0 : (size_t)row;
                    rowi[k] = row;
                    coli[k] = c;
                    lri[k] = lr;
                    ov[k] = P.accumulate ? *reinterpret_cast<const float4*>(P.dx + rr * P.lddx + c)
                                         : make_float4(0.f, 0.f, 0.f, 0.f);
                    if (P.has_cellb) {
                        const float* g = Cb.gates + rr * Cb.ldg + c;
                        gi[k] = *reinterpret_cast<const float4*>(g);
                        gf[k] = *reinterpret_cast<const float4*>(g + cn);
                        gg[k] = *reinterpret_cast<const float4*>(g + 2 * cn);
                        go[k] = *reinterpret_cast<const float4*>(g + 3 * cn);
                        cnew[k] = *reinterpret_cast<const float4*>(Cb.c_new + rr * Cb.ldc + c);
                        cprev[k] = *reinterpret_cast<const float4*>(Cb.c_prev + rr * Cb.ldc + c);
                        dcv[k] = *reinterpret_cast<const float4*>(Cb.dc + rr * Cb.lddc + c);
                    }
                }
#pragma unroll
                for (int k = 0; k < kIt; ++k) {
                    if (rowi[k] < 0) continue;
                    const float4 v = *reinterpret_cast<const float4*>(E + lri[k] * es + coli[k]);
                    const float tot[4] = {ov[k].x + v.x, ov[k].y + v.y, ov[k].z + v.z, ov[k].w + v.w};
                    *reinterpret_cast<float4*>(P.dx + (size_t)rowi[k] * P.lddx + coli[k]) =
                        make_float4(tot[0], tot[1], tot[2], tot[3]);
                    if (P.has_cellb) {
                        const float gi_[4] = {gi[k].x, gi[k].y, gi[k].z, gi[k].w};
                        const float gf_[4] = {gf[k].x, gf[k].y, gf[k].z, gf[k].w};
                        const float gg_[4] = {gg[k].x, gg[k].y, gg[k].z, gg[k].w};
                        const float go_[4] = {go[k].x, go[k].y, go[k].z, go[k].w};
                        const float cn_[4] = {cnew[k].x, cnew[k].y, cnew[k].z, cnew[k].w};
                        const float cp_[4] = {cprev[k].x, cprev[k].y, cprev[k].z, cprev[k].w};
                        const float dc_[4] = {dcv[k].x, dcv[k].y, dcv[k].z, dcv[k].w};
                        float o0[4], o1[4], o2[4], o3[4], o4[4];
#pragma unroll
                        for (int q = 0; q < 4; ++q) {
                            const float tc = tanh_fast(cn_[q]);
                            const float d = tot[q] * go_[q] * (1.0f - tc * tc) + dc_[q];
                            o0[q] = d * gg_[q] * gi_[q] * (1.0f - gi_[q]);
                            o1[q] = d * cp_[q] * gf_[q] * (1.0f - gf_[q]);
                            o2[q] = d * gi_[q] * (1.0f - gg_[q] * gg_[q]);
                            o3[q] = tot[q] * tc * go_[q] * (1.0f - go_[q]);
                            o4[q] = d * gf_[q];
                        }
                        if (!(Cb.g3 && Cb.skip_f32)) {
                            float* g = Cb.gates + (size_t)rowi[k] * Cb.ldg + coli[k];
                            *reinterpret_cast<float4*>(g) = make_float4(o0[0], o0[1], o0[2], o0[3]);
                            *reinterpret_cast<float4*>(g + cn) = make_float4(o1[0], o1[1], o1[2], o1[3]);
                            *reinterpret_cast<float4*>(g + 2 * cn) = make_float4(o2[0], o2[1], o2[2], o2[3]);
                            *reinterpret_cast<float4*>(g + 3 * cn) = make_float4(o3[0], o3[1], o3[2], o3[3]);
                        }
                        *reinterpret_cast<float4*>(Cb.dc + (size_t)rowi[k] * Cb.lddc + coli[k]) =
                            make_float4(o4[0], o4[1], o4[2], o4[3]);
                        if (Cb.g3) {
                            const int64_t ir = (int64_t)Cb.g3_row0 + rowi[k];
                            const int c0 = coli[k];
                            img_store4(Cb.g3 + img_off(ir, c0 >> 4, Cb.g3_steps), c0, o0[0], o0[1], o0[2], o0[3]);
                            img_store4(Cb.g3 + img_off(ir, (cn + c0) >> 4, Cb.g3_steps), cn + c0, o1[0], o1[1], o1[2], o1[3]);
                            img_store4(Cb.g3 + img_off(ir, (2 * cn + c0) >> 4, Cb.g3_steps), 2 * cn + c0, o2[0], o2[1], o2[2], o2[3]);
                            img_store4(Cb.g3 + img_off(ir, (3 * cn + c0) >> 4, Cb.g3_steps), 3 * cn + c0, o3[0], o3[1], o3[2], o3[3]);
                        }
                    }
                }
            }
        }
        MARL_TS();
        float* tmp = D;
        D = E;
        E = tmp;
    }
}

int panel_bwd_blocks(int m) { return (int)cdiv(m, kPanelRows); }
int panel_chain_blocks(int na, int nb) { return na >= 1 && na <= kPanelRows ? (int)cdiv(nb, kPanelRows / na) : 0; }
int panel_chain_by_batch(int na) { return na >= 1 && na <= kPanelRows ? kPanelRows / na : 0; }

struct PanelBwdPlan {
    int waves, maxc;
    size_t lds;
    unsigned pblocks, cblocks;
    bool retried;
};
static int panel_bwd_plan(PanelBwdProb& p, PanelBwdPlan& pl) {
    int waves = 8, pmax = 0, nmax = 0, prm = 0;
    pl.retried = false;
    const PanelBwdLayer& Ll = p.layer[p.nlayers - 1];
    bool tail_lds = (Ll.k_in & 3) == 0 && (p.lddx & 3) == 0 &&
                    (!p.has_cellb || ((p.cellb.n & 3) == 0 && (p.cellb.ldg & 3) == 0 && (p.cellb.ldc & 3) == 0 &&
                                      (p.cellb.lddc & 3) == 0 && p.cellb.n == Ll.k_in)) &&
                    true;
plan:
    waves = 8;
    pmax = nmax = prm = 0;
    p.tail_lds = tail_lds ? 1 : 0;
    for (int l = 0; l < p.nlayers; ++l) {
        const PanelBwdLayer& L = p.layer[l];
        if (!L.wtfrag) {
            set_error("panel backward: layer %d has no fragment-order copy of its transposed weight", l);
            return MARL_EINVAL;
        }
        if (L.wgroups != panel_frag_groups(L.n)) {
            set_error("panel backward: layer %d's weight copy has %d groups, its width %d needs %d", l, L.wgroups, L.n,
                      panel_frag_groups(L.n));
            return MARL_ELIMIT;
        }
        if (L.n > 64 * kBwdMaxCols) {
            set_error("panel backward: LayerNorm width %d > %d", L.n, 64 * kBwdMaxCols);
            return MARL_ELIMIT;
        }
        int w = panel_waves_for(L.n, L.k_in);
        if (w < 0) w = kPanelMaxWaves;
        waves = w > waves ? w : waves;
        nmax = L.n > nmax ? L.n : nmax;
        pmax = panel_stride(L.n) > pmax ? panel_stride(L.n) : pmax;
        if ((l + 1 < p.nlayers || tail_lds) && panel_stride(L.k_in) > pmax) pmax = panel_stride(L.k_in);
        prm += 2 * L.n;
    }
    if (waves > kPanelMaxWaves) waves = kPanelMaxWaves;
    p.off_e = kPanelRows * pmax;
    p.off_prm = 2 * kPanelRows * pmax;
    p.off_colp = p.off_prm + prm + 16;
    p.off_part = p.off_colp + waves * 2 * nmax;
    p.off_rowmap = p.off_part + (waves - 1) * 512;
    p.off_mix = p.off_rowmap + kPanelRows;
    if (p.mix && p.agg_at <= 0) {
        set_error("panel backward: a mixing matrix needs the in-panel aggregation");
        return MARL_ELIMIT;
    }
    if (p.gate.pos && (!p.mix || p.by_batch * p.g_na * p.g_na > kPanelRows * kPanelRows)) {
        set_error("panel backward: a position gate needs a base matrix and by_batch * agents^2 <= %d",
                  kPanelRows * kPanelRows);
        return MARL_ELIMIT;
    }
    const size_t lds = (size_t)(p.off_mix + (p.mix ? kPanelRows * kPanelRows : 0)) * sizeof(float);
    if (p.agg_at > 0 && (p.by_batch < 1 || p.g_na * p.by_batch > kPanelRows || p.agg_at >= p.nlayers ||
                         !panel_chain_supported(p.g_na, p.layer[p.agg_at].n, 256))) {
        set_error("panel backward: in-panel message mean outside its range");
        return MARL_ELIMIT;
    }
    if (lds > kPanelMaxLds && tail_lds) {
        tail_lds = false;
        pl.retried = true;
        goto plan;
    }
    if (lds > kPanelMaxLds) {
        set_error("panel backward: shape outside its range");
        return MARL_ELIMIT;
    }
    pl.pblocks = p.by_batch > 0 ? (unsigned)cdiv(p.g_nb, p.by_batch) : (unsigned)cdiv(p.m, kPanelRows);
    p.cellb_img_done = p.has_cellb && p.cellb.g3 && tail_lds;
    p.cell_vec4 = p.has_cell && lstm_bwd_vec4_ok(p.cell);
    p.cell_img_done = p.has_cell && p.cell.g3 && p.cell_vec4;
    if (!p.cellb_img_done) p.cellb.skip_f32 = 0;
    if (!p.cell_img_done) p.cell.skip_f32 = 0;
    pl.waves = waves;
    pl.lds = lds;
    pl.maxc = nmax <= 128 ? 2 : kBwdMaxCols;
    pl.cblocks = 0;
    if (p.has_cell) {
        p.panel_blocks = (int)pl.pblocks;
        pl.cblocks = (unsigned)cdiv(p.cell_rows * (p.cell_vec4 ? p.cell.n / 4 : p.cell.n), 64 * waves);
    }
    return MARL_OK;
}

int launch_panel_bwd(PanelBwdProb& p, hipStream_t st) {
    PanelBwdPlan pl;
    MARL_TRY(panel_bwd_plan(p, pl));
    const int waves = pl.waves, maxc = pl.maxc;
    const size_t lds = pl.lds;
    const unsigned pblocks = pl.pblocks;
    static bool raised = false;
    if (!raised) {
        const void* kerns[12] = {reinterpret_cast<const void*>(panel_bwd_kernel<false, 2>),
                                reinterpret_cast<const void*>(panel_bwd_kernel<true, 2>),
                                reinterpret_cast<const void*>(panel_bwd_kernel<false, kBwdMaxCols>),
                                reinterpret_cast<const void*>(panel_bwd_kernel<true, kBwdMaxCols>),
                                reinterpret_cast<const void*>(panel_bwd_kernel<false, 2, true>),
                                reinterpret_cast<const void*>(panel_bwd_kernel<true, 2, true>),
                                reinterpret_cast<const void*>(panel_bwd_kernel<false, kBwdMaxCols, true>),
                                reinterpret_cast<const void*>(panel_bwd_kernel<true, kBwdMaxCols, true>),
                                reinterpret_cast<const void*>(panel_bwd_kernel<false, 2, true, true>),
                                reinterpret_cast<const void*>(panel_bwd_kernel<true, 2, true, true>),
                                reinterpret_cast<const void*>(panel_bwd_kernel<false, kBwdMaxCols, true, true>),
                                reinterpret_cast<const void*>(panel_bwd_kernel<true, kBwdMaxCols, true, true>)};
        for (const void* kf : kerns)
            MARL_HIP_CHECK(hipFuncSetAttribute(kf, hipFuncAttributeMaxDynamicSharedMemorySize, (int)kPanelMaxLds));
        raised = true;
    }
    prof_before(4, st);
#ifdef MARL_KERNEL_TS
    static long long* d_ts = nullptr;
    static int calls = 0;
    const int rec = ts_begin(&d_ts, calls++);
    p.ts = rec ? d_ts : nullptr;
#endif
    const unsigned cblocks = pl.cblocks;
    if (p.mix) {
        const dim3 blk(64 * waves);
        if (p.gate.pos) {
            if (p.has_cell && maxc == 2)
                hipLaunchKernelGGL((panel_bwd_kernel<true, 2, true, true>), dim3(pblocks + cblocks), blk, lds, st, p);
            else if (p.has_cell)
                hipLaunchKernelGGL((panel_bwd_kernel<true, kBwdMaxCols, true, true>), dim3(pblocks + cblocks), blk, lds,
                                   st, p);
            else if (maxc == 2)
                hipLaunchKernelGGL((panel_bwd_kernel<false, 2, true, true>), dim3(pblocks), blk, lds, st, p);
            else
                hipLaunchKernelGGL((panel_bwd_kernel<false, kBwdMaxCols, true, true>), dim3(pblocks), blk, lds, st, p);
        } else if (p.has_cell && maxc == 2)
            hipLaunchKernelGGL((panel_bwd_kernel<true, 2, true>), dim3(pblocks + cblocks), blk, lds, st, p);
        else if (p.has_cell)
            hipLaunchKernelGGL((panel_bwd_kernel<true, kBwdMaxCols, true>), dim3(pblocks + cblocks), blk, lds, st, p);
        else if (maxc == 2)
            hipLaunchKernelGGL((panel_bwd_kernel<false, 2, true>), dim3(pblocks), blk, lds, st, p);
        else
            hipLaunchKernelGGL((panel_bwd_kernel<false, kBwdMaxCols, true>), dim3(pblocks), blk, lds, st, p);
    } else if (p.has_cell) {
        if (maxc == 2)
            hipLaunchKernelGGL((panel_bwd_kernel<true, 2>), dim3(pblocks + cblocks), dim3(64 * waves), lds, st, p);
        else
            hipLaunchKernelGGL((panel_bwd_kernel<true, kBwdMaxCols>), dim3(pblocks + cblocks), dim3(64 * waves), lds, st, p);
    } else if (maxc == 2) {
        hipLaunchKernelGGL((panel_bwd_kernel<false, 2>), dim3(pblocks), dim3(64 * waves), lds, st, p);
    } else {
        hipLaunchKernelGGL((panel_bwd_kernel<false, kBwdMaxCols>), dim3(pblocks), dim3(64 * waves), lds, st, p);
    }
    prof_after(4, st);
    MARL_LAUNCH_CHECK();
#ifdef MARL_KERNEL_TS
    if (rec) {
        fprintf(stderr, "[ts] panel_bwd layers %d waves %d lds %zu cell %d cellb %d tail_lds %d\n", p.nlayers, waves, lds,
                p.has_cell, p.has_cellb, p.tail_lds);
        ts_report("panel_bwd", d_ts, waves);
    }
#endif
    return MARL_OK;
}

}

#include "../../include/marl_hip_panelops.h"

using namespace marl;

namespace {

constexpr int kApiMaxWidth = 64 * kPanelMaxCols;
static float g_here[4];

bool al16(const void* p) { return (reinterpret_cast<uintptr_t>(p) & 15) == 0; }
int round4(int v) { return (v + 3) & ~3; }

bool vec_ok(const void* p, int ld, int cols) { return p && al16(p) && (ld & 3) == 0 && ld >= round4(cols); }

LstmBwdArgs cell_args(const marl_panel_cell& c) {
    LstmBwdArgs a{};
    a.dh = c.dh, a.dc = c.dc, a.gates = c.gates, a.c_prev = c.c_prev, a.c_new = c.c_new;
    a.lddh = c.lddh, a.lddc = c.lddc, a.ldg = c.ldg, a.ldc = c.ldc, a.n = c.n;
    a.g3 = static_cast<char*>(c.g3), a.g3_row0 = c.g3_row0, a.g3_steps = c.g3_steps, a.skip_f32 = c.skip_f32;
    return a;
}

struct FragJobs {
    PermBatch transposes, frags;
    size_t floats;
};

int check_grouping(const char* who, int& by_batch, int g_na, int g_nb, int m, int agg_at, int nlayers,
                   const float* mix) {
    if (by_batch < 0) by_batch = panel_chain_by_batch(g_na);
    if (by_batch > 0) {
        if (g_na < 1 || g_nb < 1 || (int64_t)g_na * g_nb != m) {
            set_error("%s: by_batch needs g_na, g_nb >= 1 and m == g_na * g_nb", who);
            return MARL_EINVAL;
        }
        if (by_batch * g_na > kPanelRows) {
            set_error("%s: by_batch * g_na = %d > %d panel rows", who, by_batch * g_na, kPanelRows);
            return MARL_ELIMIT;
        }
    }
    if (mix && agg_at <= 0) {
        set_error("%s: a mixing matrix needs the in-panel aggregation (agg_at > 0)", who);
        return MARL_ELIMIT;
    }
    if (agg_at < 0 || (agg_at > 0 && (by_batch < 1 || agg_at >= nlayers))) {
        set_error("%s: agg_at needs by_batch > 0 and 0 < agg_at < nlayers", who);
        return MARL_EINVAL;
    }
    return MARL_OK;
}

int build_fwd(const marl_panel_fwd_prob* probs, int count, float* scratch, size_t scratch_bytes, bool plan_only,
              PanelFwdBatch& b, FragJobs& jobs) {
    if (!probs || count < 1 || count > 2) {
        set_error("marl_panel_fwd: one or two problems");
        return MARL_EINVAL;
    }
    b = PanelFwdBatch{};
    b.count = count;
    jobs.transposes.count = jobs.frags.count = 0;
    jobs.floats = 0;
    for (int i = 0; i < count; ++i) {
        const marl_panel_fwd_prob& q = probs[i];
        PanelFwdProb& p = b.p[i];
        if (q.sample || q.explore || q.gate_pos) {
            set_error("marl_panel_fwd: the sampling epilogue, exploration controls and the position gate are not served here");
            return MARL_EINVAL;
        }
        if (q.nlayers < 1 || q.nlayers > kPanelMaxLayers || q.m < 1 || q.k0 < 1) {
            set_error("marl_panel_fwd: 1..%d layers, m >= 1, k0 >= 1", kPanelMaxLayers);
            return MARL_EINVAL;
        }
        if (!vec_ok(q.x, q.ldx, q.k0)) {
            set_error("marl_panel_fwd: x must be 16-byte aligned with ldx %% 4 == 0 and ldx >= round4(k0)");
            return MARL_EINVAL;
        }
        int by_batch = q.by_batch;
        MARL_TRY(check_grouping("marl_panel_fwd", by_batch, q.g_na, q.g_nb, q.m, q.agg_at, q.nlayers, q.mix));
        if (q.agg_na < 0 || (q.agg_na > 0 && (q.agg_nb < 1 || (int64_t)q.agg_na * q.agg_nb != q.m))) {
            set_error("marl_panel_fwd: the staged mean needs m == agg_na * agg_nb");
            return MARL_EINVAL;
        }
        if (q.xbar && q.agg_na > 0 && !al16(q.xbar)) {
            set_error("marl_panel_fwd: xbar must be 16-byte aligned");
            return MARL_EINVAL;
        }
        p.x = q.x, p.ldx = q.ldx, p.k0 = q.k0, p.agg_na = q.agg_na, p.agg_nb = q.agg_nb, p.xbar = q.xbar;
        p.m = q.m, p.nlayers = q.nlayers;
        p.by_batch = by_batch, p.g_na = q.g_na, p.g_nb = q.g_nb, p.agg_at = q.agg_at, p.ld_xbar = q.ld_xbar;
        p.mix = q.mix;
        int kin = q.k0;
        for (int l = 0; l < q.nlayers; ++l) {
            const marl_panel_layer& s = q.layer[l];
            if (s.n < 1 || s.n > kApiMaxWidth || (l > 0 && kin > kApiMaxWidth)) {
                set_error("marl_panel_fwd: layer %d width %d outside 1..%d", l, s.n, kApiMaxWidth);
                return MARL_ELIMIT;
            }
            if (!s.w) {
                set_error("marl_panel_fwd: layer %d has no weight (null fragment source)", l);
                return MARL_EINVAL;
            }
            if (s.ldw < kin || !s.bias || !s.gamma || !s.beta || !s.a || s.lda < s.n || (s.z && s.ldz < s.n)) {
                set_error("marl_panel_fwd: layer %d: null vector or output, or a leading dimension below its width", l);
                return MARL_EINVAL;
            }
            if (s.a3 && ((s.n & 3) || (s.a3_col0 & 3) || s.a3_col0 < 0 || s.a3_row0 < 0 ||
                         s.a3_col0 + s.n > 16 * s.a3_steps)) {
                set_error("marl_panel_fwd: layer %d: an image needs n and a3_col0 multiples of 4 inside a3_steps", l);
                return MARL_EINVAL;
            }
            if (l == q.agg_at && l > 0 && q.xbar && !vec_ok(q.xbar, q.ld_xbar, kin)) {
                set_error("marl_panel_fwd: xbar must be 16-byte aligned with ld_xbar %% 4 == 0 and >= round4(width)");
                return MARL_EINVAL;
            }
            PanelLayer& d = p.layer[l];
            d.wgroups = panel_frag_groups(kin);
            d.bias = s.bias, d.gamma = s.gamma, d.beta = s.beta, d.n = s.n;
            d.z = s.z, d.ldz = s.ldz, d.stats = s.stats, d.a = s.a, d.lda = s.lda;
            d.a3 = static_cast<char*>(s.a3), d.a3_row0 = s.a3_row0, d.a3_steps = s.a3_steps, d.a3_col0 = s.a3_col0;
            const size_t fl = panel_frag_floats(s.n, kin);
            if (plan_only) {
                d.wfrag = g_here;
            } else {
                d.wfrag = scratch + jobs.floats;
                PermDesc pd{};
                pd.src = s.w, pd.dst = scratch + jobs.floats, pd.rows = s.n, pd.cols = kin;
                pd.rd = 1, pd.rs1 = s.ldw, pd.cd = 1, pd.cs1 = 1, pd.frag = d.wgroups;
                jobs.frags.d[jobs.frags.count++] = pd;
            }
            jobs.floats += fl;
            kin = s.n;
        }
    }
    if (!plan_only && (!scratch || !al16(scratch) || scratch_bytes < jobs.floats * sizeof(float))) {
        set_error("marl_panel_fwd: scratch too small or misaligned (%zu bytes needed)", jobs.floats * sizeof(float));
        return MARL_ESIZE;
    }
    return MARL_OK;
// ... 234 lines not shown
```

marlclassification_amd/csrc/sample.h:

```cpp
#pragma once

#include "common.h"

namespace marl {

__device__ __forceinline__ float sample_silu(float y) { return silu_fast(y); }

struct Philox4 {
    uint32_t x, y, z, w;
};
__device__ __forceinline__ Philox4 philox4x32_10(uint64_t key, uint64_t ctr_hi, uint32_t c0, uint32_t c1) {
    uint32_t k0 = (uint32_t)key, k1 = (uint32_t)(key >> 32);
    Philox4 c{c0, c1, (uint32_t)ctr_hi, (uint32_t)(ctr_hi >> 32)};
#pragma unroll
    for (int i = 0; i < 10; ++i) {
        const uint32_t hi0 = __umulhi(0xD2511F53u, c.x), lo0 = 0xD2511F53u * c.x;
        const uint32_t hi1 = __umulhi(0xCD9E8D57u, c.z), lo1 = 0xCD9E8D57u * c.z;
        c = Philox4{hi1 ^ c.y ^ k0, lo1, hi0 ^ c.w ^ k1, lo0};
        k0 += 0x9E3779B9u;
        k1 += 0xBB67AE85u;
    }
    return c;
}
__device__ __forceinline__ float philox_u01(uint32_t v) { return ((float)(v >> 8) + 0.5f) * (1.0f / 16777216.0f); }

template <int MAXA, int NU = 8>
__device__ __forceinline__ void sample_logits_chunk(const SampleArgs& A, const float (&a)[NU], int base,
                                                    float (&p)[MAXA], int lane) {
#pragma unroll
    for (int j0 = 0; j0 < MAXA; j0 += 4) {
        if (j0 < A.nA) {
            float wv[4][NU];
#pragma unroll
            for (int jj = 0; jj < 4; ++jj) {
                const int j = j0 + jj < A.nA ? j0 + jj : A.nA - 1;
                const float* wj = A.w1 + (size_t)j * A.ldw;
#pragma unroll
                for (int u = 0; u < NU; ++u) {
                    const int k = base + lane + 64 * u;
                    const float v = wj[k < A.nla ? k : 0];
                    wv[jj][u] = k < A.nla ? v : 0.f;
                }
            }
#pragma unroll
            for (int jj = 0; jj < 4; ++jj) {
                float s = 0.f;
#pragma unroll
                for (int u = 0; u < NU; ++u) s += a[u] * wv[jj][u];
                p[j0 + jj] += s;
            }
        }
    }
}

template <int MAXA, int NU = 8>
__device__ __forceinline__ void sample_row_logits_at(const SampleArgs& A, const float* ar, float (&p)[MAXA], int lane) {
#pragma unroll
    for (int j = 0; j < MAXA; ++j) p[j] = 0.f;
    for (int base = 0; base < (NU < 8 ? 1 : A.nla); base += 512) {
        float a[NU];
#pragma unroll
        for (int u = 0; u < NU; ++u) {
            const int k = base + lane + 64 * u;
            const float v = ar[k < A.nla ? k : 0];
            a[u] = k < A.nla ? v : 0.f;
        }
        sample_logits_chunk<MAXA, NU>(A, a, base, p, lane);
    }
}
template <int MAXA>
__device__ __forceinline__ void sample_row_logits(const SampleArgs& A, int r, float (&p)[MAXA], int lane) {
    sample_row_logits_at<MAXA>(A, A.a_pol + (size_t)r * A.ld_a, p, lane);
}

template <int MAXA>
struct SamplePre {
    float b1[MAXA];
    float nz[MAXA];
    uint64_t ctr;
    int pi0, pi1, forced;
    bool pe_fast;
    float4 qb, qw[4], qg, qbt;
};
__device__ __forceinline__ bool sample_pe_fast(const SampleArgs& A) {
    const uintptr_t al = (uintptr_t)A.pe_W | (uintptr_t)A.pe_b | (uintptr_t)A.pe_gamma | (uintptr_t)A.pe_beta |
                         (uintptr_t)A.pe_z | (uintptr_t)A.pe_out;
    return A.pe_W && A.step_logp && (al & 15) == 0 && A.pe_nd <= 256 && ((A.pe_nd | A.pe_ldz | A.pe_ldo) & 3) == 0 &&
           (A.pe_col0 & 3) == 0;
}
template <int MAXA>
__device__ __forceinline__ void sample_prefetch_row(const SampleArgs& A, int r, int lane, SamplePre<MAXA>& S) {
#pragma unroll
    for (int j = 0; j < MAXA; ++j) S.b1[j] = A.b1[j < A.nA ? j : A.nA - 1];
    if (A.noise) {
        const float* nr = A.noise + (size_t)r * A.nA;
#pragma unroll
        for (int j = 0; j < MAXA; ++j) S.nz[j] = nr[j < A.nA ? j : A.nA - 1];
    } else {
#pragma unroll
        for (int j = 0; j < MAXA; ++j) S.nz[j] = 1.0f;
    }
    S.ctr = A.rng_ctr + (A.rng_off_dev ? (*A.rng_off_dev << 16) : 0ull);
    S.pi0 = S.pi1 = S.forced = 0;
    if (A.step_logp) {
        S.pi0 = A.pos_in[r * 2];
        S.pi1 = A.pos_in[r * 2 + 1];
        if (A.forced) S.forced = (int)A.forced[r];
    }
    S.pe_fast = false;
}
template <int MAXA>
__device__ __forceinline__ void sample_prefetch_pe(const SampleArgs& A, int lane, SamplePre<MAXA>& S) {
    S.pe_fast = sample_pe_fast(A);
    if (S.pe_fast) {
        const int j4 = 4 * lane < A.pe_nd ? 4 * lane : 0;
        S.qb = *reinterpret_cast<const float4*>(A.pe_b + j4);
        S.qg = *reinterpret_cast<const float4*>(A.pe_gamma + j4);
        S.qbt = *reinterpret_cast<const float4*>(A.pe_beta + j4);
#pragma unroll
        for (int q = 0; q < 4; ++q) S.qw[q] = *reinterpret_cast<const float4*>(A.pe_W + 4 * (j4 + q));
    }
}
template <int MAXA, bool PE = true>
__device__ __forceinline__ void sample_prefetch(const SampleArgs& A, int r, int lane, SamplePre<MAXA>& S) {
    sample_prefetch_row<MAXA>(A, r, lane, S);
    if (PE) sample_prefetch_pe<MAXA>(A, lane, S);
}

__device__ __forceinline__ float explore_logit(const SampleArgs& A, float z) { return z * A.ex_inv_tau; }
__device__ __forceinline__ float explore_mix(const SampleArgs& A, float s) { return fmaf(A.ex_keep, s, A.ex_floor); }

template <int MAXA, bool EXPLORE = false>
__device__ __forceinline__ void sample_finish(const SampleArgs& A, int r, float (&p)[MAXA], int lane,
                                              const SamplePre<MAXA>& S) {
    float mx = -INFINITY;
#pragma unroll
    for (int j = 0; j < MAXA; ++j) {
        if (j < A.nA) {
            p[j] = wave_sum(p[j]) + S.b1[j];
            if (EXPLORE) p[j] = explore_logit(A, p[j]);
            mx = fmaxf(mx, p[j]);
        } else {
            p[j] = 0.f;
        }
    }
    float den = 0.f;
#pragma unroll
    for (int j = 0; j < MAXA; ++j)
        if (j < A.nA) {
            p[j] = expf(p[j] - mx);
            den += p[j];
        }
    int act = 0;
    float best = -INFINITY, pa = 0.f;
#pragma unroll
    for (int j = 0; j < MAXA; ++j)
        if (j < A.nA) {
            p[j] = p[j] / den;
            if (EXPLORE) {
                p[j] = explore_mix(A, p[j]);
                if (A.ex_greedy && p[j] > best) {
                    best = p[j];
                    act = j;
                }
            }
            if (A.noise) {
                const float sc = p[j] / S.nz[j];
                if (sc > best) {
                    best = sc;
                    act = j;
                }
            }
        }
    if (!A.noise && A.rng_on) {
#pragma unroll
        for (int j0 = 0; j0 < MAXA; j0 += 4) {
            if (j0 < A.nA) {
                const Philox4 u = philox4x32_10(A.rng_seed, S.ctr, (uint32_t)r, (uint32_t)(j0 >> 2));
                const uint32_t uv[4] = {u.x, u.y, u.z, u.w};
#pragma unroll
                for (int jj = 0; jj < 4; ++jj) {
                    if (j0 + jj < A.nA) {
                        const float sc = p[j0 + jj] / -__logf(philox_u01(uv[jj]));
                        if (sc > best) {
                            best = sc;
                            act = j0 + jj;
                        }
                    }
                }
            }
        }
    }
    if (!A.step_logp) {
        if (lane == 0)
#pragma unroll
            for (int j = 0; j < MAXA; ++j)
                if (j < A.nA) A.probs[(size_t)r * A.nA + j] = p[j];
        return;
    }
    if (A.forced) {
        const int fa = S.forced;
        act = fa < 0 ? 0 : (fa >= A.nA ? A.nA - 1 : fa);
    }
    int mv0 = 0, mv1 = 0;
#pragma unroll
    for (int j = 0; j < MAXA; ++j)
        if (j == act) {
            pa = p[j];
            mv0 = A.table[j][0];
            mv1 = A.table[j][1];
        }
    const int pi0 = S.pi0, pi1 = S.pi1;
    const int q0 = pi0 + mv0, q1 = pi1 + mv1;
    const bool ok = q0 >= 0 && q0 + A.f < A.H && q1 >= 0 && q1 + A.f < A.W;
    const int n0 = ok ? q0 : pi0, n1 = ok ? q1 : pi1;
    if (lane == 0) {
#pragma unroll
        for (int j = 0; j < MAXA; ++j)
            if (j < A.nA) A.probs[(size_t)r * A.nA + j] = p[j];
        A.actions_i32[r] = act;
        A.step_logp[r] = logf(pa);
        A.pos_out[r * 2] = n0;
        A.pos_out[r * 2 + 1] = n1;
        if (A.step_pos) {
            A.step_pos[(size_t)r * 2] = n0;
            A.step_pos[(size_t)r * 2 + 1] = n1;
        }
        if (A.step_actions) A.step_actions[r] = act;
    }
    if (A.pe_W) {
        const float p0 = (float)n0 / (float)A.H, p1 = (float)n1 / (float)A.W;
        const int nd = A.pe_nd;
        if (lane == 0 && A.pe_npos) {
            A.pe_npos[(size_t)r * 4] = p0;
            A.pe_npos[(size_t)r * 4 + 1] = p1;
        }
        if (S.pe_fast) {
            const bool on = 4 * lane < nd;
            const float b4[4] = {S.qb.x, S.qb.y, S.qb.z, S.qb.w}, g4[4] = {S.qg.x, S.qg.y, S.qg.z, S.qg.w};
            const float t4[4] = {S.qbt.x, S.qbt.y, S.qbt.z, S.qbt.w};
            float v[4], sm = 0.f;
#pragma unroll
            for (int q = 0; q < 4; ++q) {
                v[q] = on ? b4[q] + p0 * S.qw[q].x + p1 * S.qw[q].y : 0.f;
                sm += v[q];
            }
            if (on) *reinterpret_cast<float4*>(A.pe_z + (size_t)r * A.pe_ldz + 4 * lane) = make_float4(v[0], v[1], v[2], v[3]);
            const float mean = wave_sum(sm) / (float)nd;
            float qq = 0.f;
#pragma unroll
            for (int q = 0; q < 4; ++q) {
                const float dd = on ? v[q] - mean : 0.f;
                qq += dd * dd;
            }
            const float rstd = 1.0f / sqrtf(wave_sum(qq) / (float)nd + 1e-5f);
            if (lane == 0 && A.pe_stats) {
                A.pe_stats[(size_t)r * 2] = mean;
                A.pe_stats[(size_t)r * 2 + 1] = rstd;
            }
            if (on) {
                float o[4];
#pragma unroll
                for (int q = 0; q < 4; ++q) o[q] = sample_silu((v[q] - mean) * rstd * g4[q] + t4[q]);
                *reinterpret_cast<float4*>(A.pe_out + (size_t)r * A.pe_ldo + 4 * lane) = make_float4(o[0], o[1], o[2], o[3]);
                if (A.pe_img) {
                    const int col = A.pe_col0 + 4 * lane;
// ... 44 lines not shown
```

Before: 9.439 million agent-env-steps/s.

## Specialize panel forward/backward kernels on compile-time model shapes

Adds compile-time network descriptors (PanelNet, PanelBwdNet) so the panel forward and backward kernels can be instantiated with fixed layer widths, wave counts and LDS offsets. Static GEMM slices are fully unrolled with the K-split computed at compile time. A plan flag selects the static path when chain mode is on without comm or exploration and the model matches. Also hints the sampler with the fixed action count and tweaks the LayerNorm variance accumulation. This removes runtime shape branches and address arithmetic, at the cost of more kernel instantiations, larger code, and a fallback whenever the shapes do not match.

```diff
diff --git a/marlclassification_amd/csrc/common.h b/marlclassification_amd/csrc/common.h
--- a/marlclassification_amd/csrc/common.h
+++ b/marlclassification_amd/csrc/common.h
@@ -551,6 +551,7 @@
 int panel_chain_supported(int na, int n_msg, int threads);
 int panel_supported(int k0, int n0, int n1);
 int panel_sample_supported(int n_actions);
+int panel_static_model(int n_b, int n_a, int nm2, int n_m, int n_mo, int nla, int n_actions, int n_d);
 int launch_panel_fwd(PanelFwdBatch& b, hipStream_t st, bool explore = false);
 
 struct LstmBwdArgs {
diff --git a/marlclassification_amd/csrc/episode.hip b/marlclassification_amd/csrc/episode.hip
--- a/marlclassification_amd/csrc/episode.hip
+++ b/marlclassification_amd/csrc/episode.hip
@@ -575,6 +575,7 @@
     bool panels_bwd;
     bool chain;
     bool panel_sample;
+    bool panel_static;
     bool g3_lstm;
     bool g3_tn, g3_tn_pipe;
     bool g3_tn_cell;
@@ -644,6 +645,8 @@
     p.chain = p.panels_bwd && panel_chain_supported(d.na, d.n_m, 256) && tune_get("panel_chain", 1) != 0 &&
               (!opt.comm || d.n_b <= 384);
     p.panel_sample = p.chain && env_sample && panel_sample_supported(d.nA);
+    p.panel_static = p.chain && !opt.comm && !opt.explore.on &&
+                     panel_static_model(d.n_b, d.n_a, d.nm2, d.n_m, d.n_mo, d.nla, d.nA, d.n_d);
     p.sample = p.chain ? (p.panel_sample ? SAMPLE_EPILOGUE : SAMPLE_OWN)
                        : (p.panels && !opt.explore.on ? SAMPLE_RIDE : SAMPLE_OWN);
     p.comm_form = opt.comm ? (p.chain ? 5 : p.panels ? 3 : 4) : p.chain ? 0 : p.panels ? 1 : 2;
@@ -2815,6 +2818,7 @@
     else if (!strcmp(key, "comm_range")) *value = plan.comm_range;
     else if (!strcmp(key, "panel_chain")) *value = plan.chain;
     else if (!strcmp(key, "panel_sample")) *value = plan.panel_sample;
+    else if (!strcmp(key, "panel_static")) *value = plan.panel_static;
     else if (!strcmp(key, "explore")) *value = plan.explore;
     else if (!strcmp(key, "class_loss")) *value = plan.class_loss;
     else if (!strcmp(key, "soft_targets")) *value = plan.soft_targets;
diff --git a/marlclassification_amd/csrc/panel.hip b/marlclassification_amd/csrc/panel.hip
--- a/marlclassification_amd/csrc/panel.hip
+++ b/marlclassification_amd/csrc/panel.hip
@@ -9,6 +9,10 @@
 
 __device__ __forceinline__ void lds_barrier() {
     asm volatile("s_waitcnt lgkmcnt(0)\n\ts_barrier" ::: "memory");
+}
+__device__ __forceinline__ float mul_rn(float a, float b) {
+#pragma clang fp contract(off)
+    return a * b;
 }
 __device__ __forceinline__ float silu_p(float y) { return silu_fast(y); }
 __device__ __forceinline__ float silu_grad_p(float y) { return silu_grad_fast(y); }
@@ -88,6 +92,143 @@
     return ks < 1 ? 1 : ks;
 }
 
+constexpr int panel_kper_c(int K16, int ks) { return (((K16 + ks - 1) / ks) + 15) & ~15; }
+constexpr int panel_ksplit_c(int K, int nt, int nwaves) {
+    const int K16 = (K + 15) & ~15, want = (K16 + 63) / 64;
+    int ks = nwaves / nt;
+    ks = ks < want ? ks : want;
+    return ks < 1 ? 1 : ks;
+}
+constexpr int panel_stride_c(int k) { return ((k + 15) & ~15) + 4; }
+constexpr int cmax(int a, int b) { return a > b ? a : b; }
+
+struct PanelDyn {
+    static constexpr bool kStatic = false, kByBatch = false;
+    static constexpr int kLayers = kPanelMaxLayers, kSoft = 0, kWaves = 0, kK0 = 0, kAggAt = 0, kKLast = 0;
+    static constexpr int off_e = 0, off_prm = 0, off_colp = 0, off_part = 0, off_rowmap = 0;
+    static constexpr int n(int) { return 0; }
+    static constexpr int k(int) { return 0; }
+};
+template <int WAVES, int K0, int AGG_AT, int SOFT, int... N>
+struct PanelNet {
+    static constexpr bool kStatic = true, kByBatch = AGG_AT > 0;
+    static constexpr int kLayers = (int)sizeof...(N), kSoft = SOFT, kWaves = WAVES, kK0 = K0, kAggAt = AGG_AT;
+    static constexpr int n(int l) {
+        constexpr int w[] = {N...};
+        return w[l];
+    }
+    static constexpr int k(int l) { return l == 0 ? K0 : n(l - 1); }
+    static constexpr int s0(int layers) {
+        int v = kPanelRows * panel_stride_c(K0);
+        for (int l = 1; l < layers; l += 2) v = cmax(v, kPanelRows * panel_stride_c(n(l)));
+        return v;
+    }
+    static constexpr int s1(int layers) {
+        int v = 0;
+        for (int l = 0; l < layers; l += 2) v = cmax(v, kPanelRows * panel_stride_c(n(l)));
+        return v;
+    }
+    static constexpr bool ok() {
+        for (int l = 0; l < kLayers; ++l) {
+            const int nt = (n(l) + 31) >> 5, K16 = (k(l) + 15) & ~15, ks = panel_ksplit_c(k(l), nt, WAVES);
+            if (nt * ks > WAVES || (ks - 1) * panel_kper_c(K16, ks) >= K16) return false;
+            if ((n(l) & 15) || (k(l) & 15) || n(l) > 64 * kPanelMaxCols) return false;
+        }
+        return WAVES >= 4 && WAVES <= kPanelMaxWaves && (SOFT == 0 || (s0(SOFT) == s0(kLayers) && s1(SOFT) == s1(kLayers)));
+    }
+};
+template <int WAVES, int AGG_AT, int KLAST, int... N>
+struct PanelBwdNet {
+    static constexpr bool kStatic = true, kByBatch = true;
+    static constexpr int kLayers = (int)sizeof...(N), kSoft = 0, kWaves = WAVES, kAggAt = AGG_AT, kKLast = KLAST;
+    static constexpr int n(int l) {
+        constexpr int w[] = {N...};
+        return w[l];
+    }
+    static constexpr int k(int l) { return l + 1 < kLayers ? n(l + 1) : KLAST; }
+    static constexpr int nmax() {
+        int v = 0;
+        for (int l = 0; l < kLayers; ++l) v = cmax(v, n(l));
+        return v;
+    }
+    static constexpr int pmax() {
+        int v = 0;
+        for (int l = 0; l < kLayers; ++l) v = cmax(v, cmax(panel_stride_c(n(l)), panel_stride_c(k(l))));
+        return v;
+    }
+    static constexpr int prm() {
+        int v = 0;
+        for (int l = 0; l < kLayers; ++l) v += 2 * n(l);
+        return v;
+    }
+    static constexpr int off_e = kPanelRows * pmax(), off_prm = 2 * kPanelRows * pmax(), off_colp = off_prm + prm() + 16;
+    static constexpr int off_part = off_colp + WAVES * 2 * nmax(), off_rowmap = off_part + (WAVES - 1) * 512;
+    static constexpr bool ok() {
+        for (int l = 0; l < kLayers; ++l) {
+            const int nt = (k(l) + 31) >> 5, n16 = (n(l) + 15) & ~15, ks = panel_ksplit_c(n(l), nt, WAVES);
+            if (nt > WAVES || (ks - 1) * panel_kper_c(n16, ks) >= n16) return false;
+            if ((n(l) & 15) || (k(l) & 15)) return false;
+        }
+        return WAVES >= 8 && WAVES <= kPanelMaxWaves && nmax() <= 128 && (KLAST & 3) == 0;
+    }
+};
+
+template <int K16, int KS, int KPER>
+__device__ __forceinline__ void panel_gemm_st(f32x4 (&acc)[2], const float* in, int stride,
+                                              const float* __restrict__ wfrag, int j, int s, int lane) {
+    constexpr int groups = K16 >> 4, last0 = (KS - 1) * KPER;
+    static_assert(last0 < K16 && (KPER & 15) == 0, "slice plan");
+    const int quad = lane >> 4, l16 = lane & 15;
+    const int kbeg = __builtin_amdgcn_readfirstlane(s * KPER);
+    const float* arow = in + l16 * stride + 4 * quad + kbeg;
+    const int g0 = __builtin_amdgcn_readfirstlane(j * groups + (kbeg >> 4));
+    const float* wb = wfrag + (size_t)g0 * 512;
+    const unsigned lo = 4u * (unsigned)lane;
+#pragma unroll
+    for (int r = 0; r < 4; ++r) acc[0][r] = acc[1][r] = 0.f;
+#pragma unroll
+    for (int c = 0; c < (KPER + 63) / 64; ++c) {
+        if (last0 + 64 * c < K16 || kbeg + 64 * c < K16) {
+            float4 b0[4], b1[4];
+#pragma unroll
+            for (int i = 0; i < 4; ++i) {
+                if (64 * c + 16 * i < KPER) {
+                    b0[i] = *reinterpret_cast<const float4*>(wb + 2048 * c + 512 * i + lo);
+                    b1[i] = *reinterpret_cast<const float4*>(wb + 2048 * c + 512 * i + 256 + lo);
+                }
+            }
+#pragma unroll
+            for (int i = 0; i < 4; ++i) {
+                if (64 * c + 16 * i < KPER && (last0 + 64 * c + 16 * i < K16 || kbeg + 64 * c + 16 * i < K16)) {
+                    const float4 a = *reinterpret_cast<const float4*>(arow + 64 * c + 16 * i);
+                    acc[0] = __builtin_amdgcn_mfma_f32_16x16x4f32(a.x, b0[i].x, acc[0], 0, 0, 0);
+                    acc[1] = __builtin_amdgcn_mfma_f32_16x16x4f32(a.x, b1[i].x, acc[1], 0, 0, 0);
+                    acc[0] = __builtin_amdgcn_mfma_f32_16x16x4f32(a.y, b0[i].y, acc[0], 0, 0, 0);
+                    acc[1] = __builtin_amdgcn_mfma_f32_16x16x4f32(a.y, b1[i].y, acc[1], 0, 0, 0);
+                    acc[0] = __builtin_amdgcn_mfma_f32_16x16x4f32(a.z, b0[i].z, acc[0], 0, 0, 0);
+                    acc[1] = __builtin_amdgcn_mfma_f32_16x16x4f32(a.z, b1[i].z, acc[1], 0, 0, 0);
+                    acc[0] = __builtin_amdgcn_mfma_f32_16x16x4f32(a.w, b0[i].w, acc[0], 0, 0, 0);
+                    acc[1] = __builtin_amdgcn_mfma_f32_16x16x4f32(a.w, b1[i].w, acc[1], 0, 0, 0);
+                }
+            }
+        }
+    }
+}
+
+template <class SH, bool BWD, int L = 0>
+__device__ __forceinline__ void panel_gemm_layer(int l, f32x4 (&acc)[2], const float* in, int stride,
+                                                 const float* __restrict__ wfrag, int j, int s, int lane) {
+    if constexpr (SH::kStatic && L < SH::kLayers) {
+        if (l == L) {
+            constexpr int K = BWD ? SH::n(L) : SH::k(L), nout = BWD ? SH::k(L) : SH::n(L);
+            constexpr int K16 = (K + 15) & ~15, ks = panel_ksplit_c(K, (nout + 31) >> 5, SH::kWaves);
+            panel_gemm_st<K16, ks, panel_kper_c(K16, ks)>(acc, in, stride, wfrag, j, s, lane);
+        } else {
+            panel_gemm_layer<SH, BWD, L + 1>(l, acc, in, stride, wfrag, j, s, lane);
+        }
+    }
+}
+
 template <int NC>
 __device__ __forceinline__ void panel_ln_rows(const PanelLayer& Lr, float* outp, int ys, int n, const float* lgamma,
                                               const float* lbeta, const int* rowmap, int wave, int nwaves, int lane)
@@ -117,14 +258,15 @@
                 if (Lr.z && row >= 0 && c < n) Lr.z[(size_t)row * Lr.ldz + c] = v[u];
             }
             const float mean = wave_sum(sm) * inv_n;
-            float q = 0.f;
 #pragma unroll
             for (int u = 0; u < NC; ++u) {
                 const int c = lane + 64 * u;
-                const float d = c < n ? v[u] - mean : 0.f;
-                v[u] = d;
-                q += d * d;
-            }
+                v[u] = c < n ? v[u] - mean : 0.f;
+            }
+            static_assert(NC >= 2, "column slots");
+            float q = fmaf(v[0], v[0], mul_rn(v[1], v[1]));
+#pragma unroll
+            for (int u = 2; u < NC; ++u) q = fmaf(v[u], v[u], q);
             const float rstd = 1.0f / sqrtf(wave_sum(q) * inv_n + 1e-5f);
             float* arow = Lr.a + (size_t)(row < 0 ? 0 : row) * Lr.lda;
 #pragma unroll
@@ -151,7 +293,7 @@
     }
 }
 
-template <int MAXA, bool UNI, bool EXPLORE = false>
+template <int MAXA, bool UNI, bool EXPLORE = false, int NLA = 0>
 __device__ __forceinline__ void panel_sample_rows(const SampleArgs& A0, const float* outp, int ys, const int* rowmap,
                                                   int wave, int nwaves, int lane) {
     for (int lr = __builtin_amdgcn_readfirstlane(wave); lr < kPanelRows; lr += nwaves) {
@@ -162,6 +304,10 @@
         int zero = 0;
         asm volatile("" : "+s"(zero));
         const SampleArgs& A = (&A0)[zero];
+        if (NLA > 0) {
+            __builtin_assume(A.nA == MAXA);
+            __builtin_assume(A.nla == NLA);
+        }
         float p[MAXA];
         SamplePre<MAXA> S;
         sample_prefetch_row<MAXA>(A, row, ln, S);
@@ -179,34 +325,27 @@
             S.pi1 = __builtin_amdgcn_readfirstlane(S.pi1);
             S.forced = __builtin_amdgcn_readfirstlane(S.forced);
         }
-        sample_prefetch_pe<MAXA>(A, ln, S);
+        sample_prefetch_pe<MAXA, (NLA > 0)>(A, ln, S);
         sample_finish<MAXA, EXPLORE>(A, row, p, ln, S);
     }
 }
 
-template <int SAMPLE, bool MIX = false, bool EPI = false, bool GATE = false, bool EXPLORE = false>
-__global__ __launch_bounds__(768, 6) void panel_fwd_kernel(const PanelFwdBatch B) {
-    extern __shared__ __attribute__((aligned(16))) float lds[];
-    if (!EPI && SAMPLE > 0 && (int)blockIdx.x >= B.panel_blocks) {
-        const int r = ((int)blockIdx.x - B.panel_blocks) * (int)(blockDim.x >> 6) + (int)(threadIdx.x >> 6);
-        if (r >= B.sample.R) return;
-        constexpr int MAXA = SAMPLE > 0 ? SAMPLE : 4;
-        float p[MAXA];
-        SamplePre<MAXA> S;
-        sample_prefetch<MAXA, false>(B.sample, r, threadIdx.x & 63, S);
-        sample_row_logits<MAXA>(B.sample, r, p, threadIdx.x & 63);
-        sample_finish<MAXA>(B.sample, r, p, threadIdx.x & 63, S);
-        return;
-    }
-    const PanelFwdProb& P = B.p[blockIdx.y];
+struct PanelDynLay {
+    static constexpr int panel1 = 0, red = 0, part = 0, prm = 0;
+};
+template <class SH, class LY, int SAMPLE, bool MIX, bool EPI, bool GATE, bool EXPLORE>
+__device__ __forceinline__ void panel_fwd_body(const PanelFwdBatch& B, const PanelFwdProb& P, float* lds) {
+    constexpr bool ST = SH::kStatic;
     const int m0 = blockIdx.x * kPanelRows;
-    const int bpb = P.by_batch;
-    if (bpb ? (int)blockIdx.x * bpb >= P.g_nb : m0 >= P.m) return;
-    const int tid = threadIdx.x, lane = tid & 63, wave = tid >> 6, nwaves = blockDim.x >> 6;
-    int* rowmap = reinterpret_cast<int*>(lds + B.off_red);
+    const int bpb = ST && !SH::kByBatch ? 0 : P.by_batch;
+    if ((ST ? SH::kByBatch : bpb != 0) ? (int)blockIdx.x * bpb >= P.g_nb : m0 >= P.m) return;
+#define PANEL_NT (ST ? 64u * SH::kWaves : blockDim.x)
+#define PANEL_NL (ST && SH::kSoft == 0 ? SH::kLayers : P.nlayers)
+    const int tid = threadIdx.x, lane = tid & 63, wave = tid >> 6, nwaves = PANEL_NT >> 6;
+    int* rowmap = reinterpret_cast<int*>(lds + (ST ? LY::red : B.off_red));
     if (tid < kPanelRows) {
         int r = m0 + tid < P.m ? m0 + tid : -1;
-        if (bpb) {
+        if (ST ? SH::kByBatch : bpb != 0) {
             const int a = tid / bpb, b = (int)blockIdx.x * bpb + (tid - a * bpb);
             r = (a < P.g_na && b < P.g_nb) ? a * P.g_nb + b : -1;
         }
@@ -219,14 +358,15 @@
 #endif
     MARL_TS();
     float* X = lds;
-    float* Y = lds + B.off_panel1;
-    float* part = lds + B.off_part;
-    float* prm = lds + B.off_prm;
+    float* Y = lds + (ST ? LY::panel1 : B.off_panel1);
+    float* part = lds + (ST ? LY::part : B.off_part);
+    float* prm = lds + (ST ? LY::prm : B.off_prm);
     float pv[kPanelMaxLayers][3];
 #pragma unroll
     for (int l = 0; l < kPanelMaxLayers; ++l) {
         pv[l][0] = pv[l][1] = pv[l][2] = 0.f;
-        if (l < P.nlayers && tid < P.layer[l].n) {
+        if (ST && l >= SH::kLayers) continue;
+        if (l < PANEL_NL && tid < (ST ? SH::n(l) : P.layer[l].n)) {
             pv[l][0] = P.layer[l].bias[tid];
             pv[l][1] = P.layer[l].gamma[tid];
             pv[l][2] = P.layer[l].beta[tid];
@@ -241,13 +381,13 @@
     }
 
     {
-        const int k0 = P.k0, xs = panel_stride(k0), K16 = (k0 + 15) & ~15;
+        const int k0 = ST ? SH::kK0 : P.k0, xs = panel_stride(k0), K16 = (k0 + 15) & ~15;
         const int c4 = K16 >> 2;
         const int K4 = (k0 + 3) & ~3;
-        if (!GATE && P.agg_na > 0) {
+        if (!GATE && !ST && P.agg_na > 0) {
             const int na = P.agg_na, nb = P.agg_nb;
             const float den = (float)(na - 1);
-            for (int e = tid; e < kPanelRows * c4; e += blockDim.x) {
+            for (int e = tid; e < kPanelRows * c4; e += PANEL_NT) {
                 const int lr = e / c4, k = (e % c4) * 4;
                 const int r = rowmap[lr];
                 float4 v = make_float4(0.f, 0.f, 0.f, 0.f);
@@ -284,7 +424,7 @@
             float4 xv[2];
 #pragma unroll
             for (int it = 0; it < 2; ++it) {
-                const int e = tid + it * (int)blockDim.x;
+                const int e = tid + it * (int)PANEL_NT;
                 xv[it] = make_float4(0.f, 0.f, 0.f, 0.f);
                 if (e < kPanelRows * c4) {
                     const int lr = e / c4, k = (e % c4) * 4;
@@ -294,13 +434,13 @@
             }
 #pragma unroll
             for (int it = 0; it < 2; ++it) {
-                const int e = tid + it * (int)blockDim.x;
+                const int e = tid + it * (int)PANEL_NT;
                 if (e < kPanelRows * c4) {
                     const int lr = e / c4, k = (e % c4) * 4;
                     *reinterpret_cast<float4*>(X + lr * xs + k) = xv[it];
                 }
             }
-            for (int e = tid + 2 * (int)blockDim.x; e < kPanelRows * c4; e += blockDim.x) {
+            for (int e = tid + 2 * blockDim.x; e < kPanelRows * c4; e += PANEL_NT) {
                 const int lr = e / c4, k = (e % c4) * 4;
                 const int r = rowmap[lr];
                 float4 v = make_float4(0.f, 0.f, 0.f, 0.f);
@@ -310,17 +450,18 @@
         }
     }
     {
-        int off = 0;
+        int poff = 0;
 #pragma unroll
         for (int l = 0; l < kPanelMaxLayers; ++l) {
-            if (l < P.nlayers) {
-                const int n = P.layer[l].n;
+            if (ST && l >= SH::kLayers) continue;
+            if (l < PANEL_NL) {
+                const int n = ST ? SH::n(l) : P.layer[l].n;
                 if (tid < n) {
-                    prm[off + tid] = pv[l][0];
-                    prm[off + n + tid] = pv[l][1];
-                    prm[off + 2 * n + tid] = pv[l][2];
-                }
-                off += 3 * n;
+                    prm[poff + tid] = pv[l][0];
+                    prm[poff + n + tid] = pv[l][1];
+                    prm[poff + 2 * n + tid] = pv[l][2];
+                }
+                poff += 3 * n;
             }
         }
     }
@@ -330,28 +471,33 @@
     lds_barrier();
     MARL_TS();
 
-    int prm_off = 0, K = P.k0;
-    for (int l = 0; l < P.nlayers; ++l) {
+    int prm_off = 0, K = ST ? SH::kK0 : P.k0;
+    constexpr int kUnroll = ST ? SH::kLayers : 1;
+#pragma unroll kUnroll
+    for (int l = 0; l < (ST ? SH::kLayers : PANEL_NL); ++l) {
+        if (ST && SH::kSoft > 0 && l >= SH::kSoft && PANEL_NL <= SH::kSoft) break;
         const PanelLayer Lr = P.layer[l];
+        const int n = ST ? SH::n(l) : Lr.n;
         const float* lbias = prm + prm_off;
-        const float* lgamma = lbias + Lr.n;
-        const float* lbeta = lgamma + Lr.n;
-        prm_off += 3 * Lr.n;
+        const float* lgamma = lbias + n;
+        const float* lbeta = lgamma + n;
+        prm_off += 3 * n;
         float* in = (l & 1) ? Y : X;
         float* outp = (l & 1) ? X : Y;
         const int K16 = (K + 15) & ~15;
         const int stride = panel_stride(K);
-        if (l > 0 && l == P.agg_at) {
+        if (l > 0 && l == (ST ? SH::kAggAt : P.agg_at)) {
             const int c4 = K16 >> 2, K4 = (K + 3) & ~3, na = P.g_na;
             const float den = (float)(na - 1);
             float4 v[2];
 #pragma unroll
             for (int it = 0; it < 2; ++it) {
-                const int e = tid + it * (int)blockDim.x;
+                const int e = tid + it * (int)PANEL_NT;
                 v[it] = make_float4(0.f, 0.f, 0.f, 0.f);
                 if (e < kPanelRows * c4) {
                     const int lr = e / c4, k = (e - lr * c4) * 4;
-                    const int a = lr / bpb, i = lr - a * bpb;
+                    const int bd = ST && !SH::kByBatch ? 1 : bpb;
+                    const int a = lr / bd, i = lr - a * bd;
                     if (MIX) {
                         if (a < na) {
                             const float* crow = lds + B.off_mix + (GATE ? i * na + a : a) * na;
@@ -386,7 +532,7 @@
             lds_barrier();
 #pragma unroll
             for (int it = 0; it < 2; ++it) {
-                const int e = tid + it * (int)blockDim.x;
+                const int e = tid + it * (int)PANEL_NT;
                 if (e < kPanelRows * c4) {
                     const int lr = e / c4, k = (e - lr * c4) * 4;
                     *reinterpret_cast<float4*>(in + lr * stride + k) = v[it];
@@ -397,15 +543,19 @@
             }
             lds_barrier();
         }
-        const int n = Lr.n, nt = (n + 31) >> 5;
+        const int nt = (n + 31) >> 5;
         const int ks = panel_ksplit(K, nt, nwaves);
         const int j = wave % nt, s = wave / nt;
         const bool active = s < ks;
-        const int kper = (((K16 + ks - 1) / ks) + 15) & ~15;
-        const int kbeg = s * kper;
-        const int kend = kbeg + kper < K16 ? kbeg + kper : K16;
         f32x4 acc[2];
-        if (active) panel_gemm(acc, in, stride, Lr.wfrag, Lr.wgroups, j, kbeg, kend, lane);
+        if constexpr (ST) {
+            if (active) panel_gemm_layer<SH, false>(l, acc, in, stride, Lr.wfrag, j, s, lane);
+        } else {
+            const int kper = (((K16 + ks - 1) / ks) + 15) & ~15;
+            const int kbeg = s * kper;
+            const int kend = kbeg + kper < K16 ? kbeg + kper : K16;
+            if (active) panel_gemm(acc, in, stride, Lr.wfrag, Lr.wgroups, j, kbeg, kend, lane);
+        }
         MARL_TS();
         panel_ksum(acc, part, nt, ks, j, s, lane, active);
         MARL_TS();
@@ -415,20 +565,20 @@
 #pragma unroll
             for (int t = 0; t < 2; ++t) {
                 const int col = j * 32 + 16 * t + l16;
-                const bool cv = col < n;
+                const bool cv = (ST && (n & 31) == 0) || col < n;
                 const float bv = cv ? lbias[col] : 0.f;
 #pragma unroll
                 for (int r = 0; r < 4; ++r) {
                     const int lr = 4 * quad + r;
                     const float zv = cv ? acc[t][r] + bv : 0.f;
-                    if (col < n16) outp[lr * ys + col] = zv;
+                    if ((ST && (n & 31) == 0) || col < n16) outp[lr * ys + col] = zv;
                 }
             }
         }
         MARL_TS();
         lds_barrier();
         MARL_TS();
-        if (n <= B.ln_narrow_max)
+        if (n <= (ST ? 128 : B.ln_narrow_max))
             panel_ln_rows<2>(Lr, outp, ys, n, lgamma, lbeta, rowmap, wave, nwaves, lane);
         else
             panel_ln_rows<kPanelMaxCols>(Lr, outp, ys, n, lgamma, lbeta, rowmap, wave, nwaves, lane);
@@ -437,11 +587,51 @@
         MARL_TS();
         K = n;
     }
-    if (EPI && (int)(&P - B.p) + 1 == B.epi_prob) {
+    if (EPI && (ST || (int)blockIdx.y + 1 == B.epi_prob)) {
         constexpr int MAXA = SAMPLE > 0 ? SAMPLE : 4;
-        panel_sample_rows<MAXA, MIX || EXPLORE, EXPLORE>(B.sample, (P.nlayers & 1) ? Y : X, panel_stride(K), rowmap, wave, nwaves, lane);
+        panel_sample_rows<MAXA, MIX || EXPLORE || ST, EXPLORE, ST ? SH::n(ST ? SH::kLayers - 1 : 0) : 0>(
+            B.sample, (PANEL_NL & 1) ? Y : X, panel_stride(K), rowmap, wave, nwaves, lane);
         MARL_TS();
     }
+}
+
+#undef PANEL_NT
+#undef PANEL_NL
+
+template <int SAMPLE, bool MIX = false, bool EPI = false, bool GATE = false, bool EXPLORE = false>
+__global__ __launch_bounds__(768, 6) 
+void panel_fwd_kernel(const PanelFwdBatch B) {
+    extern __shared__ __attribute__((aligned(16))) float lds[];
+    if (!EPI && SAMPLE > 0 && (int)blockIdx.x >= B.panel_blocks) {
+        const int r = ((int)blockIdx.x - B.panel_blocks) * (int)(blockDim.x >> 6) + (int)(threadIdx.x >> 6);
+        if (r >= B.sample.R) return;
+        constexpr int MAXA = SAMPLE > 0 ? SAMPLE : 4;
+        float p[MAXA];
+        SamplePre<MAXA> S;
+        sample_prefetch<MAXA, false>(B.sample, r, threadIdx.x & 63, S);
+        sample_row_logits<MAXA>(B.sample, r, p, threadIdx.x & 63);
+        sample_finish<MAXA>(B.sample, r, p, threadIdx.x & 63, S);
+        return;
+    }
+    panel_fwd_body<PanelDyn, PanelDynLay, SAMPLE, MIX, EPI, GATE, EXPLORE>(B, B.p[blockIdx.y], lds);
+}
+
+template <class CH, class PO>
+struct PanelFwdLay {
+    static_assert(CH::ok() && PO::ok() && CH::kWaves == PO::kWaves && CH::kByBatch && !PO::kByBatch, "static panel nets");
+    static constexpr int waves = CH::kWaves;
+    static constexpr int panel1 = cmax(CH::s0(CH::kLayers), PO::s0(PO::kLayers));
+    static constexpr int red = panel1 + cmax(CH::s1(CH::kLayers), PO::s1(PO::kLayers));
+    static constexpr int part = red + (kPanelMaxWaves + 1) * 32, prm = part + (waves - 1) * 512;
+};
+template <class CH, class PO, bool EPI>
+__global__ __launch_bounds__(768, 6) void panel_fwd_static_kernel(const PanelFwdBatch B) {
+    extern __shared__ __attribute__((aligned(16))) float lds[];
+    using LY = PanelFwdLay<CH, PO>;
+    if (blockIdx.y == 0)
+        panel_fwd_body<CH, LY, 0, false, false, false, false>(B, B.p[0], lds);
+    else
+        panel_fwd_body<PO, LY, EPI ? 4 : 0, false, EPI, false, false>(B, B.p[1], lds);
 }
 
 constexpr size_t kPanelMaxLds = 144 * 1024;
@@ -561,6 +751,62 @@
     return MARL_OK;
 }
 
+using PanelChainNet = PanelNet<12, 256, 2, 2, 128, 64, 128, 96>;
+using PanelPolicyNet = PanelNet<12, 256, 0, 0, 384>;
+using PanelFwdStaticLay = PanelFwdLay<PanelChainNet, PanelPolicyNet>;
+using PanelBwdChainNet = PanelBwdNet<8, 2, 256, 96, 128, 64, 128>;
+using PanelBwdDecNet = PanelBwdNet<8, 0, 64, 96, 128>;
+static_assert(PanelBwdChainNet::ok() && PanelBwdDecNet::ok(), "static panel nets");
+constexpr int kPanelStaticActions = 4;
+
+static bool panel_static_env() {
+    static const bool on = [] {
+        const char* v = getenv("MARL_PANEL_STATIC");
+        return !(v && v[0] == '0');
+    }();
+    return on;
+}
+
+int panel_static_model(int n_b, int n_a, int nm2, int n_m, int n_mo, int nla, int n_actions, int n_d) {
+    using C = PanelChainNet;
+    return panel_static_env() && n_b == C::kK0 && nm2 == C::n(0) && n_m == C::n(1) && nm2 == C::n(2) && n_mo == C::n(3) &&
+           n_a == PanelPolicyNet::kK0 && nla == PanelPolicyNet::n(0) && n_actions == kPanelStaticActions &&
+           (n_d & 3) == 0 && n_d <= 256;
+}
+
+template <class SH>
+static bool panel_fwd_matches(const PanelFwdProb& p, int layers) {
+    if (p.nlayers != layers || p.k0 != SH::kK0 || p.agg_na != 0 || p.mix || p.gate.pos) return false;
+    if (SH::kByBatch ? p.by_batch < 1 : p.by_batch != 0) return false;
+    if (p.agg_at != (layers > SH::kAggAt ? SH::kAggAt : 0)) return false;
+    for (int l = 0; l < layers; ++l)
+        if (p.layer[l].n != SH::n(l) || p.layer[l].wgroups != panel_frag_groups(SH::k(l))) return false;
+    return true;
+}
+static bool panel_pe_fast_host(const SampleArgs& A) {
+    const uintptr_t al = (uintptr_t)A.pe_W | (uintptr_t)A.pe_b | (uintptr_t)A.pe_gamma | (uintptr_t)A.pe_beta |
+                         (uintptr_t)A.pe_z | (uintptr_t)A.pe_out;
+    return A.pe_W && A.step_logp && (al & 15) == 0 && A.pe_nd <= 256 && ((A.pe_nd | A.pe_ldz | A.pe_ldo) & 3) == 0 &&
+           (A.pe_col0 & 3) == 0;
+}
+static bool panel_fwd_static_ok(const PanelFwdBatch& b, const PanelFwdPlan& pl, bool explore) {
+    using LY = PanelFwdStaticLay;
+    if (!panel_static_env() || explore || pl.mixed || pl.gated || b.count != 2 || b.has_sample) return false;
+    if (!panel_fwd_matches<PanelChainNet>(b.p[0], PanelChainNet::kLayers) &&
+        !panel_fwd_matches<PanelChainNet>(b.p[0], PanelChainNet::kSoft))
+        return false;
+    if (!panel_fwd_matches<PanelPolicyNet>(b.p[1], 1)) return false;
+    if (pl.waves != LY::waves || b.off_panel1 != LY::panel1 || b.off_red != LY::red || b.off_part != LY::part ||
+        b.off_prm != LY::prm || b.ln_narrow_max != 128)
+        return false;
+    if (b.epi_prob) {
+        const SampleArgs& A = b.sample;
+        if (b.epi_prob != 2 || A.nA != kPanelStaticActions || A.nla != PanelPolicyNet::n(0)) return false;
+        if (A.pe_W && !panel_pe_fast_host(A)) return false;
+    }
+    return true;
+}
+
 int launch_panel_fwd(PanelFwdBatch& b, hipStream_t st, bool explore) {
     PanelFwdPlan pl;
     MARL_TRY(panel_fwd_plan(b, pl));
@@ -570,7 +816,9 @@
     const bool mixed = pl.mixed, gated = pl.gated;
     static bool raised = false;
     if (!raised) {
-        const void* kerns[11] = {reinterpret_cast<const void*>(panel_fwd_kernel<0>),
+        const void* kerns[13] = {reinterpret_cast<const void*>(panel_fwd_static_kernel<PanelChainNet, PanelPolicyNet, false>),
+                                reinterpret_cast<const void*>(panel_fwd_static_kernel<PanelChainNet, PanelPolicyNet, true>),
+                                reinterpret_cast<const void*>(panel_fwd_kernel<0>),
                                 reinterpret_cast<const void*>(panel_fwd_kernel<4>),
                                 reinterpret_cast<const void*>(panel_fwd_kernel<MARL_MAX_ACTIONS>),
                                 reinterpret_cast<const void*>(panel_fwd_kernel<0, true>),
@@ -614,7 +862,15 @@
         }
     }
     prof_before(4, st);
-    if (b.epi_prob && explore) {
+    if (panel_fwd_static_ok(b, pl, explore)) {
+        b.has_sample = 0;
+        if (b.epi_prob)
+            hipLaunchKernelGGL((panel_fwd_static_kernel<PanelChainNet, PanelPolicyNet, true>),
+                               dim3(pblocks, (unsigned)b.count), dim3(64 * waves), lds, st, b);
+        else
+            hipLaunchKernelGGL((panel_fwd_static_kernel<PanelChainNet, PanelPolicyNet, false>),
+                               dim3(pblocks, (unsigned)b.count), dim3(64 * waves), lds, st, b);
+    } else if (b.epi_prob && explore) {
         b.has_sample = 0;
         if (gated)
             hipLaunchKernelGGL((panel_fwd_kernel<4, true, true, true, true>), dim3(pblocks, (unsigned)b.count),
@@ -669,11 +925,13 @@
 
 constexpr int kBwdMaxCols = kPanelMaxCols;
 
-template <bool CELL, int MAXC, bool MIX = false, bool GATE = false>
+template <class SH, bool CELL, int MAXC, bool MIX = false, bool GATE = false>
 __global__ __launch_bounds__(768, 4) void panel_bwd_kernel(const PanelBwdProb P) {
     extern __shared__ __attribute__((aligned(16))) float lds[];
+    constexpr bool ST = SH::kStatic;
+    const int nthreads = ST ? 64 * SH::kWaves : (int)blockDim.x;
     if (CELL && (int)blockIdx.x >= P.panel_blocks) {
-        const int64_t idx = (int64_t)((int)blockIdx.x - P.panel_blocks) * blockDim.x + threadIdx.x;
+        const int64_t idx = (int64_t)((int)blockIdx.x - P.panel_blocks) * nthreads + threadIdx.x;
         if (P.cell_vec4)
             lstm_cell_bwd_elem4(P.cell, P.cell_rows, idx);
         else
@@ -682,18 +940,19 @@
     }
     const int m0 = blockIdx.x * kPanelRows;
     const int bpb = P.by_batch;
-    if (bpb ? (int)blockIdx.x * bpb >= P.g_nb : m0 >= P.m) return;
-    const int tid = threadIdx.x, lane = tid & 63, wave = tid >> 6, nwaves = blockDim.x >> 6;
+    if ((ST || bpb) ? (int)blockIdx.x * bpb >= P.g_nb : m0 >= P.m) return;
+    const int tid = threadIdx.x, lane = tid & 63, wave = tid >> 6, nwaves = nthreads >> 6;
     const int quad = lane >> 4, l16 = lane & 15;
+    const int nlayers = ST ? SH::kLayers : P.nlayers;
     float* D = lds;
-    float* E = lds + P.off_e;
-    float* prm = lds + P.off_prm;
-    float* colp = lds + P.off_colp;
-    float* part = lds + P.off_part;
-    int* rowmap = reinterpret_cast<int*>(lds + P.off_rowmap);
+    float* E = lds + (ST ? SH::off_e : P.off_e);
+    float* prm = lds + (ST ? SH::off_prm : P.off_prm);
+    float* colp = lds + (ST ? SH::off_colp : P.off_colp);
+    float* part = lds + (ST ? SH::off_part : P.off_part);
+    int* rowmap = reinterpret_cast<int*>(lds + (ST ? SH::off_rowmap : P.off_rowmap));
     if (tid < kPanelRows) {
         int r = m0 + tid < P.m ? m0 + tid : -1;
-        if (bpb) {
+        if (ST || bpb) {
             const int a = tid / bpb, b = (int)blockIdx.x * bpb + (tid - a * bpb);
             r = (a < P.g_na && b < P.g_nb) ? a * P.g_nb + b : -1;
         }
@@ -706,7 +965,7 @@
     MARL_TS();
 
     float zpre[2][MAXC], mpre[2], rpre[2];
-    auto zfetch = [&](const PanelBwdLayer& L) {
+    auto zfetch = [&](const PanelBwdLayer& L, const int ln) {
 #pragma unroll
         for (int i = 0; i < 2; ++i) {
             const int lr = wave + i * nwaves;
@@ -717,17 +976,18 @@
 #pragma unroll
             for (int u = 0; u < MAXC; ++u) {
                 const int c = lane + 64 * u;
-                zpre[i][u] = c < L.n ? L.z[rr * L.ldz + c] : 0.f;
+                zpre[i][u] = c < ln ? L.z[rr * L.ldz + c] : 0.f;
             }
         }
     };
-    zfetch(P.layer[0]);
+    zfetch(P.layer[0], ST ? SH::n(0) : P.layer[0].n);
     {
         float pv[kPanelMaxLayers][2];
 #pragma unroll
         for (int l = 0; l < kPanelMaxLayers; ++l) {
             pv[l][0] = pv[l][1] = 0.f;
-            if (l < P.nlayers && tid < P.layer[l].n) {
+            if (ST && l >= SH::kLayers) continue;
+            if (l < nlayers && tid < (ST ? SH::n(l) : P.layer[l].n)) {
                 pv[l][0] = P.layer[l].gamma[tid];
                 pv[l][1] = P.layer[l].beta[tid];
             }
@@ -745,8 +1005,9 @@
         int off = 0;
 #pragma unroll
         for (int l = 0; l < kPanelMaxLayers; ++l) {
-            if (l < P.nlayers) {
-                const int n = P.layer[l].n;
+            if (ST && l >= SH::kLayers) continue;
+            if (l < nlayers) {
+                const int n = ST ? SH::n(l) : P.layer[l].n;
                 if (tid < n) {
                     prm[off + tid] = pv[l][0];
                     prm[off + n + tid] = pv[l][1];
@@ -756,13 +1017,14 @@
         }
         if (MIX && !GATE && tid < P.g_na * P.g_na) lds[P.off_mix + tid] = cmv;
         if (MIX && GATE && tid < bpb * P.g_na * P.g_na) lds[P.off_mix + tid] = cmv;
-        const int n = P.layer[0].n, ds = panel_stride(n), n16 = (n + 15) & ~15, c4 = n16 >> 2;
+        const int n = ST ? SH::n(0) : P.layer[0].n, ds = panel_stride(n), n16 = (n + 15) & ~15, c4 = n16 >> 2;
         const int n4 = (n + 3) & ~3;
-        for (int e = tid; e < kPanelRows * c4; e += blockDim.x) {
+        const int agg_na = ST ? 0 : P.agg_na;
+        for (int e = tid; e < kPanelRows * c4; e += nthreads) {
             const int lr = e / c4, k = (e % c4) * 4;
             const int r = rowmap[lr];
             float4 v = make_float4(0.f, 0.f, 0.f, 0.f);
-            if (r >= 0 && k < n4 && P.agg_na > 1) {
+            if (r >= 0 && k < n4 && agg_na > 1) {
                 const int na = P.agg_na, nb = P.agg_nb;
                 const float den = (float)(na - 1);
                 const float* base = P.da + (size_t)(r % nb) * P.ldda + k;
@@ -788,7 +1050,7 @@
                 const float4 me = *reinterpret_cast<const float4*>(P.da + (size_t)r * P.ldda + k);
                 v = make_float4((s.x - me.x) / den, (s.y - me.y) / den, (s.z - me.z) / den,
                                 (s.w - me.w) / den);
-            } else if (r >= 0 && k < n4 && P.agg_na == 0) {
+            } else if (r >= 0 && k < n4 && agg_na == 0) {
                 v = *reinterpret_cast<const float4*>(P.da + (size_t)r * P.ldda + k);
                 if (P.da2) {
                     const float4 w = *reinterpret_cast<const float4*>(P.da2 + (size_t)r * P.ldda2 + k);
@@ -803,19 +1065,21 @@
     MARL_TS();
 
     int prm_off = 0;
-    for (int l = 0; l < P.nlayers; ++l) {
+    constexpr int kUnroll = ST ? SH::kLayers : 1;
+#pragma unroll kUnroll
+    for (int l = 0; l < nlayers; ++l) {
         const PanelBwdLayer Lr = P.layer[l];
-        const int n = Lr.n, ds = panel_stride(n), n16 = (n + 15) & ~15;
+        const int n = ST ? SH::n(l) : Lr.n, ds = panel_stride(n), n16 = (n + 15) & ~15;
         const float* lgamma = prm + prm_off;
         const float* lbeta = lgamma + n;
         prm_off += 2 * n;
-        if (l > 0 && l == P.agg_at) {
+        if (l > 0 && l == (ST ? SH::kAggAt : P.agg_at)) {
             const int c4 = n16 >> 2, na = P.g_na;
             const float den = (float)(na - 1);
             float4 v[2];
 #pragma unroll
             for (int it = 0; it < 2; ++it) {
-                const int e = tid + it * (int)blockDim.x;
+                const int e = tid + it * nthreads;
                 v[it] = make_float4(0.f, 0.f, 0.f, 0.f);
                 if (e < kPanelRows * c4) {
                     const int lr = e / c4, k = (e - lr * c4) * 4;
@@ -854,7 +1118,7 @@
             lds_barrier();
 #pragma unroll
             for (int it = 0; it < 2; ++it) {
-                const int e = tid + it * (int)blockDim.x;
+                const int e = tid + it * nthreads;
                 if (e < kPanelRows * c4) {
                     const int lr = e / c4, k = (e - lr * c4) * 4;
                     *reinterpret_cast<float4*>(D + lr * ds + k) = v[it];
@@ -890,11 +1154,11 @@
                             xh[u] = dxh[u] = 0.f;
                             if (c < n) {
                                 xh[u] = (zpre[i][u] - mean) * rstd;
-                                const float dy = D[lr * ds + c] * silu_grad_p(g[u] * xh[u] + bt[u]);
-                                dxh[u] = dy * g[u];
+                                const float dy = mul_rn(D[lr * ds + c], silu_grad_p(g[u] * xh[u] + bt[u]));
+                                dxh[u] = mul_rn(dy, g[u]);
                                 s1 += dxh[u];
-                                s2 += dxh[u] * xh[u];
-                                pg[u] += dy * xh[u];
+                                s2 += mul_rn(dxh[u], xh[u]);
+                                pg[u] += mul_rn(dy, xh[u]);
                                 pb[u] += dy;
                             }
                         }
@@ -930,26 +1194,31 @@
         MARL_TS();
         lds_barrier();
         MARL_TS();
-        for (int c = tid; c < 2 * n; c += blockDim.x) {
+        for (int c = tid; c < 2 * n; c += nthreads) {
             float t = 0.f;
             for (int w = 0; w < nwaves; ++w) t += colp[(size_t)w * 2 * n + c];
             Lr.part[(size_t)blockIdx.x * 2 * n + c] = t;
         }
-        if (l + 1 < P.nlayers) zfetch(P.layer[l + 1]);
+        if (l + 1 < nlayers) zfetch(P.layer[l + 1], ST ? SH::n(l + 1 < SH::kLayers ? l + 1 : 0) : P.layer[l + 1].n);
         MARL_TS();
-        const int nout = Lr.k_in, nt = (nout + 31) >> 5;
+        const int nout = ST ? SH::k(l) : Lr.k_in, nt = (nout + 31) >> 5;
         const int ks = panel_ksplit(n, nt, nwaves);
         const int kper = (((n16 + ks - 1) / ks) + 15) & ~15;
-        const bool last = l + 1 == P.nlayers;
+        const bool last = l + 1 == nlayers;
+        const bool tail_lds = ST || P.tail_lds;
         const int es = panel_stride(nout), o16 = (nout + 15) & ~15;
         for (int t0 = 0; t0 < nt; t0 += nwaves / ks) {
             const int tiles_round = nwaves / ks;
             const int j = t0 + wave % tiles_round, s = wave / tiles_round;
             const bool active = s < ks && j < nt;
-            const int kbeg = s * kper;
-            const int kend = kbeg + kper < n16 ? kbeg + kper : n16;
             f32x4 acc[2];
-            if (active) panel_gemm(acc, D, ds, Lr.wtfrag, Lr.wgroups, j, kbeg, kend, lane);
+            if constexpr (ST) {
+                if (active) panel_gemm_layer<SH, true>(l, acc, D, ds, Lr.wtfrag, j, s, lane);
+            } else {
+                const int kbeg = s * kper;
+                const int kend = kbeg + kper < n16 ? kbeg + kper : n16;
+                if (active) panel_gemm(acc, D, ds, Lr.wtfrag, Lr.wgroups, j, kbeg, kend, lane);
+            }
             panel_ksum(acc, part, tiles_round, ks, wave % tiles_round, s, lane, active);
             if (active && s == 0) {
                 int rw[4];
@@ -963,7 +1232,7 @@
                         const int lr = 4 * quad + r;
                         const int row = rw[r];
                         const float v = col < nout ? acc[t][r] : 0.f;
-                        if (last && P.tail_lds) {
+                        if (last && tail_lds) {
                             if (col < o16) E[lr * es + col] = v;
                         } else if (last) {
                             if (col < nout && row >= 0) {
@@ -981,16 +1250,16 @@
             lds_barrier();
         }
         MARL_TS();
-        if (last && P.tail_lds) {
+        if (last && tail_lds) {
             const LstmBwdArgs& Cb = P.cellb;
-            const int c4n = nout >> 2, items = kPanelRows * c4n, cn = Cb.n;
+            const int c4n = nout >> 2, items = kPanelRows * c4n, cn = ST ? nout : Cb.n;
             constexpr int kIt = 1;
-            for (int base = 0; base < items; base += kIt * (int)blockDim.x) {
+            for (int base = 0; base < items; base += kIt * nthreads) {
                 float4 ov[kIt], gi[kIt], gf[kIt], gg[kIt], go[kIt], cnew[kIt], cprev[kIt], dcv[kIt];
                 int rowi[kIt], coli[kIt], lri[kIt];
 #pragma unroll
                 for (int k = 0; k < kIt; ++k) {
-                    const int i = base + tid + k * (int)blockDim.x;
+                    const int i = base + tid + k * nthreads;
                     const int lr = i < items ? i / c4n : 0;
                     const int c = i < items ? (i - lr * c4n) * 4 : 0;
                     const int row = i < items ? rowmap[lr] : -1;
@@ -1158,6 +1427,19 @@
     return MARL_OK;
 }
 
+template <class SH>
+static bool panel_bwd_static_ok(const PanelBwdProb& p, const PanelBwdPlan& pl) {
+    if (!panel_static_env() || p.mix || p.gate.pos || p.nlayers != SH::kLayers || p.agg_na != 0 || p.by_batch < 1 ||
+        p.agg_at != SH::kAggAt || !p.tail_lds || pl.maxc != 2 || pl.waves != SH::kWaves)
+        return false;
+    for (int l = 0; l < SH::kLayers; ++l)
+        if (p.layer[l].n != SH::n(l) || p.layer[l].k_in != SH::k(l) || p.layer[l].wgroups != panel_frag_groups(SH::n(l)))
+            return false;
+    if (p.has_cellb && p.cellb.n != SH::kKLast) return false;
+    return p.off_e == SH::off_e && p.off_prm == SH::off_prm && p.off_colp == SH::off_colp && p.off_part == SH::off_part &&
+           p.off_rowmap == SH::off_rowmap;
+}
+
 int launch_panel_bwd(PanelBwdProb& p, hipStream_t st) {
     PanelBwdPlan pl;
     MARL_TRY(panel_bwd_plan(p, pl));
@@ -1166,18 +1448,21 @@
     const unsigned pblocks = pl.pblocks;
     static bool raised = false;
     if (!raised) {
-        const void* kerns[12] = {reinterpret_cast<const void*>(panel_bwd_kernel<false, 2>),
-                                reinterpret_cast<const void*>(panel_bwd_kernel<true, 2>),
-                                reinterpret_cast<const void*>(panel_bwd_kernel<false, kBwdMaxCols>),
-                                reinterpret_cast<const void*>(panel_bwd_kernel<true, kBwdMaxCols>),
-                                reinterpret_cast<const void*>(panel_bwd_kernel<false, 2, true>),
-                                reinterpret_cast<const void*>(panel_bwd_kernel<true, 2, true>),
-                                reinterpret_cast<const void*>(panel_bwd_kernel<false, kBwdMaxCols, true>),
-                                reinterpret_cast<const void*>(panel_bwd_kernel<true, kBwdMaxCols, true>),
-                                reinterpret_cast<const void*>(panel_bwd_kernel<false, 2, true, true>),
-                                reinterpret_cast<const void*>(panel_bwd_kernel<true, 2, true, true>),
-                                reinterpret_cast<const void*>(panel_bwd_kernel<false, kBwdMaxCols, true, true>),
-                                reinterpret_cast<const void*>(panel_bwd_kernel<true, kBwdMaxCols, true, true>)};
+        const void* kerns[15] = {reinterpret_cast<const void*>(panel_bwd_kernel<PanelBwdChainNet, false, 2>),
+                                reinterpret_cast<const void*>(panel_bwd_kernel<PanelBwdChainNet, true, 2>),
+                                reinterpret_cast<const void*>(panel_bwd_kernel<PanelBwdDecNet, false, 2>),
+                                reinterpret_cast<const void*>(panel_bwd_kernel<PanelDyn, false, 2>),
+                                reinterpret_cast<const void*>(panel_bwd_kernel<PanelDyn, true, 2>),
+                                reinterpret_cast<const void*>(panel_bwd_kernel<PanelDyn, false, kBwdMaxCols>),
+                                reinterpret_cast<const void*>(panel_bwd_kernel<PanelDyn, true, kBwdMaxCols>),
+                                reinterpret_cast<const void*>(panel_bwd_kernel<PanelDyn, false, 2, true>),
+                                reinterpret_cast<const void*>(panel_bwd_kernel<PanelDyn, true, 2, true>),
+                                reinterpret_cast<const void*>(panel_bwd_kernel<PanelDyn, false, kBwdMaxCols, true>),
+                                reinterpret_cast<const void*>(panel_bwd_kernel<PanelDyn, true, kBwdMaxCols, true>),
+                                reinterpret_cast<const void*>(panel_bwd_kernel<PanelDyn, false, 2, true, true>),
+                                reinterpret_cast<const void*>(panel_bwd_kernel<PanelDyn, true, 2, true, true>),
+                                reinterpret_cast<const void*>(panel_bwd_kernel<PanelDyn, false, kBwdMaxCols, true, true>),
+                                reinterpret_cast<const void*>(panel_bwd_kernel<PanelDyn, true, kBwdMaxCols, true, true>)};
         for (const void* kf : kerns)
             MARL_HIP_CHECK(hipFuncSetAttribute(kf, hipFuncAttributeMaxDynamicSharedMemorySize, (int)kPanelMaxLds));
         raised = true;
@@ -1190,35 +1475,43 @@
     p.ts = rec ? d_ts : nullptr;
 #endif
     const unsigned cblocks = pl.cblocks;
-    if (p.mix) {
+    if (panel_bwd_static_ok<PanelBwdChainNet>(p, pl)) {
+        if (p.has_cell)
+            hipLaunchKernelGGL((panel_bwd_kernel<PanelBwdChainNet, true, 2>), dim3(pblocks + cblocks), dim3(64 * waves), lds,
+                               st, p);
+        else
+            hipLaunchKernelGGL((panel_bwd_kernel<PanelBwdChainNet, false, 2>), dim3(pblocks), dim3(64 * waves), lds, st, p);
+    } else if (!p.has_cell && panel_bwd_static_ok<PanelBwdDecNet>(p, pl)) {
+        hipLaunchKernelGGL((panel_bwd_kernel<PanelBwdDecNet, false, 2>), dim3(pblocks), dim3(64 * waves), lds, st, p);
+    } else if (p.mix) {
         const dim3 blk(64 * waves);
         if (p.gate.pos) {
             if (p.has_cell && maxc == 2)
-                hipLaunchKernelGGL((panel_bwd_kernel<true, 2, true, true>), dim3(pblocks + cblocks), blk, lds, st, p);
+                hipLaunchKernelGGL((panel_bwd_kernel<PanelDyn, true, 2, true, true>), dim3(pblocks + cblocks), blk, lds, st, p);
             else if (p.has_cell)
-                hipLaunchKernelGGL((panel_bwd_kernel<true, kBwdMaxCols, true, true>), dim3(pblocks + cblocks), blk, lds,
+                hipLaunchKernelGGL((panel_bwd_kernel<PanelDyn, true, kBwdMaxCols, true, true>), dim3(pblocks + cblocks), blk, lds,
                                    st, p);
             else if (maxc == 2)
-                hipLaunchKernelGGL((panel_bwd_kernel<false, 2, true, true>), dim3(pblocks), blk, lds, st, p);
+                hipLaunchKernelGGL((panel_bwd_kernel<PanelDyn, false, 2, true, true>), dim3(pblocks), blk, lds, st, p);
             else
-                hipLaunchKernelGGL((panel_bwd_kernel<false, kBwdMaxCols, true, true>), dim3(pblocks), blk, lds, st, p);
+                hipLaunchKernelGGL((panel_bwd_kernel<PanelDyn, false, kBwdMaxCols, true, true>), dim3(pblocks), blk, lds, st, p);
         } else if (p.has_cell && maxc == 2)
-            hipLaunchKernelGGL((panel_bwd_kernel<true, 2, true>), dim3(pblocks + cblocks), blk, lds, st, p);
+            hipLaunchKernelGGL((panel_bwd_kernel<PanelDyn, true, 2, true>), dim3(pblocks + cblocks), blk, lds, st, p);
         else if (p.has_cell)
-            hipLaunchKernelGGL((panel_bwd_kernel<true, kBwdMaxCols, true>), dim3(pblocks + cblocks), blk, lds, st, p);
+            hipLaunchKernelGGL((panel_bwd_kernel<PanelDyn, true, kBwdMaxCols, true>), dim3(pblocks + cblocks), blk, lds, st, p);
         else if (maxc == 2)
-            hipLaunchKernelGGL((panel_bwd_kernel<false, 2, true>), dim3(pblocks), blk, lds, st, p);
+            hipLaunchKernelGGL((panel_bwd_kernel<PanelDyn, false, 2, true>), dim3(pblocks), blk, lds, st, p);
         else
-            hipLaunchKernelGGL((panel_bwd_kernel<false, kBwdMaxCols, true>), dim3(pblocks), blk, lds, st, p);
+            hipLaunchKernelGGL((panel_bwd_kernel<PanelDyn, false, kBwdMaxCols, true>), dim3(pblocks), blk, lds, st, p);
     } else if (p.has_cell) {
         if (maxc == 2)
-            hipLaunchKernelGGL((panel_bwd_kernel<true, 2>), dim3(pblocks + cblocks), dim3(64 * waves), lds, st, p);
+            hipLaunchKernelGGL((panel_bwd_kernel<PanelDyn, true, 2>), dim3(pblocks + cblocks), dim3(64 * waves), lds, st, p);
         else
-            hipLaunchKernelGGL((panel_bwd_kernel<true, kBwdMaxCols>), dim3(pblocks + cblocks), dim3(64 * waves), lds, st, p);
+            hipLaunchKernelGGL((panel_bwd_kernel<PanelDyn, true, kBwdMaxCols>), dim3(pblocks + cblocks), dim3(64 * waves), lds, st, p);
     } else if (maxc == 2) {
-        hipLaunchKernelGGL((panel_bwd_kernel<false, 2>), dim3(pblocks), dim3(64 * waves), lds, st, p);
+        hipLaunchKernelGGL((panel_bwd_kernel<PanelDyn, false, 2>), dim3(pblocks), dim3(64 * waves), lds, st, p);
     } else {
-        hipLaunchKernelGGL((panel_bwd_kernel<false, kBwdMaxCols>), dim3(pblocks), dim3(64 * waves), lds, st, p);
+        hipLaunchKernelGGL((panel_bwd_kernel<PanelDyn, false, kBwdMaxCols>), dim3(pblocks), dim3(64 * waves), lds, st, p);
     }
     prof_after(4, st);
     MARL_LAUNCH_CHECK();
diff --git a/marlclassification_amd/csrc/sample.h b/marlclassification_amd/csrc/sample.h
--- a/marlclassification_amd/csrc/sample.h
+++ b/marlclassification_amd/csrc/sample.h
@@ -109,9 +109,9 @@
     }
     S.pe_fast = false;
 }
-template <int MAXA>
+template <int MAXA, bool FAST = false>
 __device__ __forceinline__ void sample_prefetch_pe(const SampleArgs& A, int lane, SamplePre<MAXA>& S) {
-    S.pe_fast = sample_pe_fast(A);
+    S.pe_fast = FAST ? A.pe_W != nullptr : sample_pe_fast(A);
     if (S.pe_fast) {
         const int j4 = 4 * lane < A.pe_nd ? 4 * lane : 0;
         S.qb = *reinterpret_cast<const float4*>(A.pe_b + j4);
```

New measurement: 9.660 million agent-env-steps/s, median of 6. 1.02x the previous value.
